# cgranerob/Land-Surface-Temperature-Super-Resolution-with-a-Scale-Invariance-Free-Neural-Approach

Measured on AMD Instinct MI355X. Metric: LST+NDVI 256x256 patches/sec (train fwd+bwd), whole job, higher is better.
Workload: dtype f32; 1 GPU; ModelB SIF-NN-SR2 (gradFTM loss) batch 64/GPU, synthetic 256x256, 1x MI355X, fwd+loss+bwd+Adam; batch_per_gpu=64, patch=256x256 (LST 64x64 + NDVI 256x256), parallelism=dp1, loss=sr2

## Files before the change

land-surface-temperature-super-resolution-with-a-scale-invariance-free-neural-approach_amd/csrc/edge_conv.h:

```cpp
#pragma once
#include "common.h"

int conv_in_fwd_blocks(int B, int H, int W);
int launch_conv_in_fwd(const float* x, const float* w, float* y, float* partials, int B, int H, int W, hipStream_t s,
                       int* nf_image = nullptr);
int launch_conv_in_wgrad(const float* x, const float* dy, float* partials, int nblk, float* dw, int B, int H, int W, hipStream_t s);
int launch_conv_out_fwd(const float* y, const float* scale, const float* shift, const float* w, const float* bias,
                        float* out, int B, int H, int W, hipStream_t s,
                        const int* nf = nullptr);
int launch_conv_out_dgrad(const float* dsr, const float* w, float* g, int B, int H, int W, hipStream_t s);
int launch_conv_out_wgrad(const float* y, const float* scale, const float* shift, const float* dsr, float* partials,
                          int nblk, float* dw, float* db, int B, int H, int W, hipStream_t s);
int launch_conv_in_wgrad_fused(const float* x, const float* g, const float* y, const float* scale, const float* shift,
                               const double* coef, float* partials, int nblk, float* dw, int B, int H, int W, hipStream_t s);
size_t conv_in_gram_scratch_floats();
int launch_conv_in_gram(const float* x, float* scratch, int B, int H, int W, hipStream_t s);
const double* conv_in_gram_result(const float* scratch);
int launch_conv_in_dz_wgrad(const float* x, const float* dz, float* partials, int nblk, int B, int H, int W, hipStream_t s);
int launch_conv_in_dw_combine(const float* partials, int nblk, const double* gram, const float* w, const double* coef, float* dw,
                              hipStream_t s);
int launch_tail_bwd_reduce(const float* y, const float* scale, const float* shift, const float* mean, const float* invstd,
                           const float* dsr, const float* w, float* wpart, float* bnpart, int nblk, int B, int H, int W,
                           hipStream_t s, int* nf = nullptr);
int launch_tail_bwd_apply(const float* y, const float* scale, const float* shift, const double* coef, const float* dsr,
                          const float* w, float* dy, int B, int H, int W, hipStream_t s);
int launch_sum_partials(const float* partials, int nblk, int n, float* out, hipStream_t s);

int launch_bn_finalize(const float* partials, int nblk, int C, double count, const float* gamma, const float* beta,
                       float* run_mean, float* run_var, float momentum, float eps, float* mean, float* invstd,
                       float* scale, float* shift, hipStream_t s,
                       int* nf = nullptr);
int launch_bn_eval_coeffs(const float* params, const float* running, float eps, float* scale, float* shift, hipStream_t s,
                          int* nf = nullptr, const int* nf_pack = nullptr);
int launch_bn_bwd_reduce(const float* g, const float* y, const float* scale, const float* shift, const float* mean,
                         const float* invstd, int C, size_t npix, float* partials, int nblk, hipStream_t s,
                         const float* gp = nullptr, int H = 0, int W = 0, float* g_out = nullptr);
int launch_bn_bwd_finalize(const float* partials, int nblk, int C, double count, const float* scale, const float* mean,
                           const float* invstd, float* dgamma, float* dbeta, double* coef, hipStream_t s,
                           const float* shift = nullptr, const float* beta = nullptr, float* coef_f = nullptr,
                           const float* xs_partials = nullptr, int xs_n = 0, float* xs_out = nullptr,
                           int frozen = 0,
                           const int* nf = nullptr);
int launch_bn_bwd_finalize2(const float* pa, int na, const float* pb, int nb, int C, double count, const float* scale,
                            const float* mean, const float* invstd, float* dgamma, float* dbeta, double* coef, hipStream_t s,
                            const float* shift = nullptr, const float* beta = nullptr, float* coef_f = nullptr, int frozen = 0,
                            const int* nf = nullptr);
int launch_bn_bwd_apply(const float* g, const float* y, const float* scale, const float* shift, const double* coef,
                        int C, size_t npix, float* dy, hipStream_t s, const float* gp = nullptr, int H = 0, int W = 0);
int launch_nbt_increment(long long* nbt, int n, hipStream_t s);

int launch_bn_frozen_stats(const float* running, float eps, float* mean, float* invstd, hipStream_t s);
int launch_conv_in_dgrad(const float* g, const float* y, const float* scale, const float* shift, const double* coef, const float* w,
                         float* dx, int B, int H, int W, hipStream_t s);

int launch_bnrelu_pool2(const float* y, const float* scale, const float* shift, float* out, int B, int H, int W, int C, hipStream_t s);
int launch_bnrelu_add(const float* p, const float* y, const float* scale, const float* shift, float* out, int C, size_t npix, hipStream_t s);
int launch_bnrelu_up2x(const float* y, const float* scale, const float* shift, float* out, int B, int Hin, int Win, int C, hipStream_t s);
int launch_pool2_bwd(const float* gp, float* g, int B, int H, int W, int C, int accumulate, hipStream_t s);
int launch_up2x_bwd(const float* gu, float* g, int B, int Hin, int Win, int C, hipStream_t s, const float* bn_y = nullptr,
                    const float* bn_scale = nullptr, const float* bn_shift = nullptr, float* bn_partials = nullptr);
int up2x_bwd_stat_rows(int B, int Hin, int Win, int C);

int launch_adam_flat(float* p, const float* g, float* m, float* v, int n, float lr, float beta1, float beta2, float eps,
                     float weight_decay, int step, float grad_scale, hipStream_t s);

int launch_adam_flat_dev(float* p, const float* g, float* m, float* v, int n, float lr, float beta1, float beta2, float eps,
                         float weight_decay, long long* step_dev, float* coef2, float grad_scale, hipStream_t s);

int launch_tiles_prepare(const float* lst, const float* ndvi, float* x, int T, int tiles_x, int win, long long lst_step_y,
                         long long lst_step_x, int lst_row, long long ndvi_step_y, long long ndvi_step_x, int ndvi_row,
                         float mean_lst, float std_lst, float mean_ndvi, float std_ndvi, int clip_ndvi, hipStream_t s);
int launch_tiles_paste(const float* sr, float* out, int T, int tiles_x, int hr, long long out_row, float mean, float std,
                       hipStream_t s);
int launch_l4pool4(const float* x, float* out, int B, int H, int W, hipStream_t s);
size_t psnr_ssim_scratch_bytes(int B, int H, int W);
int launch_psnr_ssim(const float* pred, const float* targ, int B, int H, int W, void* scratch, float* out2, hipStream_t s);
size_t psnr_ssim_masked_scratch_bytes(int B, int H, int W);
int launch_psnr_ssim_masked(const float* pred, const float* targ, const unsigned char* valid, int scale, int B, int H, int W,
                            void* scratch, float* out2, int* counts2, hipStream_t s);

size_t eval_metrics_scratch_bytes(int B, int H, int W);
int launch_eval_metrics(const float* a, const float* b, int B, int H, int W, const float* taps9, float data_range,
                        void* scratch, double* out8, hipStream_t s);
int launch_gradient_strata(const float* a, int B, int H, int W, const float* taps9, float* g, float* q2, int* counts3,
                           hipStream_t s);
size_t eval_metrics_masked_scratch_bytes(int B, int H, int W);
int launch_eval_metrics_masked(const float* a, const float* b, const unsigned char* mask, int B, int H, int W,
                               const float* taps9, float data_range, void* scratch, double* out8, int* counts5, hipStream_t s);

size_t fourier_scratch_bytes(int B, int H, int W);
int launch_fft2_attenuation(const float* img, int B, int H, int W, void* scratch, float* mag, float* spectrum, hipStream_t s);
```

land-surface-temperature-super-resolution-with-a-scale-invariance-free-neural-approach_amd/csrc/edge_conv.hip:

```cpp
#include "edge_conv.h"

namespace {

template <bool HS>
__global__ __launch_bounds__(256) void conv_in_fwd_kernel(const float* __restrict__ x, const float* __restrict__ w,
                                                          float* __restrict__ y, float* __restrict__ partials,
                                                          int B, int H, int W, int* __restrict__ nf_image) {
  __shared__ float tile[2][2 * 324];
  __shared__ float red[4][16][2];
  const int tid = threadIdx.x, lane = tid & 63, wave = tid >> 6;
  const int i = lane & 15, kq = lane >> 4;
  const int tiles_x = (W + 15) / 16, tiles_y = (H + 15) / 16, ntiles = B * tiles_x * tiles_y;
  auto stage = [&](int t, float* dst) {
    const int tx = t % tiles_x, ty = (t / tiles_x) % tiles_y, b = t / (tiles_x * tiles_y);
    const int x0 = tx * 16, y0 = ty * 16;
    for (int e = tid; e < 2 * 324; e += 256) {
      const int c = e / 324, p = e - c * 324;
      const int py = p / 18, px = p - py * 18;
      const int gy = clampi(y0 - 1 + py, 0, H - 1), gx = clampi(x0 - 1 + px, 0, W - 1);
      dst[e] = x[((size_t)(b * 2 + c) * H + gy) * W + gx];
    }
  };
  if ((int)blockIdx.x < ntiles) stage(blockIdx.x, tile[0]);
  float wa[5];
  int off[5];
#pragma unroll
  for (int j = 0; j < 5; ++j) {
    const int kk = 4 * j + kq;
    wa[j] = kk < 18 ? w[i * 18 + kk] : 0.f;
    const int c = kk >= 9 ? 1 : 0, t = kk < 18 ? kk - 9 * c : 0;
    off[j] = (kk < 18 ? c * 324 : 0) + (t / 3) * 18 + t % 3 + i;
  }
  float s1[4] = {0.f, 0.f, 0.f, 0.f}, s2[4] = {0.f, 0.f, 0.f, 0.f};
  int buf = 0;
  for (int t = blockIdx.x; t < ntiles; t += gridDim.x, buf ^= 1) {
    __syncthreads();
    if (t + (int)gridDim.x < ntiles) stage(t + gridDim.x, tile[buf ^ 1]);
    const int tx = t % tiles_x, ty = (t / tiles_x) % tiles_y, b = t / (tiles_x * tiles_y);
    const int x0 = tx * 16, y0 = ty * 16;
    const float* T = tile[buf];
    bool bad = false;
#pragma unroll
    for (int r = 0; r < 4; ++r) {
      const int row = 4 * wave + r;
      f32x4 acc = (f32x4){0.f, 0.f, 0.f, 0.f};
#pragma unroll
      for (int j = 0; j < 5; ++j) acc = __builtin_amdgcn_mfma_f32_16x16x4f32(wa[j], T[off[j] + row * 18], acc, 0, 0, 0);
      if (y0 + row < H && x0 + i < W) {
        const float4 o = as_stored4<HS>(make_float4(acc[0], acc[1], acc[2], acc[3]));
        stA4<HS>(y, ((size_t)(b * H + y0 + row) * W + x0 + i) * 16 + 4 * kq, o);
        const float ov[4] = {o.x, o.y, o.z, o.w};
#pragma unroll
        for (int q = 0; q < 4; ++q) { s1[q] += ov[q]; s2[q] = fmaf(ov[q], ov[q], s2[q]); bad = bad || nonfinite(ov[q]); }
      }
    }
    if (nf_image != nullptr && bad) nf_image[b] = 1;
  }
  if (partials != nullptr) {
#pragma unroll
    for (int q = 0; q < 4; ++q) {
#pragma unroll
      for (int m = 1; m < 16; m <<= 1) { s1[q] += __shfl_xor(s1[q], m); s2[q] += __shfl_xor(s2[q], m); }
      if (i == 0) { red[wave][4 * kq + q][0] = s1[q]; red[wave][4 * kq + q][1] = s2[q]; }
    }
    __syncthreads();
    if (tid < 32) {
      const int co = tid >> 1, j = tid & 1;
      const float s = red[0][co][j] + red[1][co][j] + red[2][co][j] + red[3][co][j];
      partials[((size_t)blockIdx.x * 16 + co) * 2 + j] = s;
    }
  }
}

template <bool FUSED, bool HS>
__global__ __launch_bounds__(256) void conv_in_wgrad_kernel(const float* __restrict__ x, const float* __restrict__ dy,
                                                            const float* __restrict__ yraw,
                                                            const float* __restrict__ scale,
                                                            const float* __restrict__ shift,
                                                            const double* __restrict__ coef,
                                                            float* __restrict__ partials, int B, int H, int W) {
  SIFSR_CHAIN_PRIO();
  __shared__ float tile[2 * 324 + 8];
  __shared__ float dyt[256 * 16];
  __shared__ float red[4][2][256];
  const int tid = threadIdx.x, lane = tid & 63, wave = tid >> 6;
  const int tiles_x = (W + 15) / 16, tiles_y = (H + 15) / 16, ntiles = B * tiles_x * tiles_y;
  const int i16 = lane & 15, k = lane >> 4;
  int offn[2];
#pragma unroll
  for (int nt = 0; nt < 2; ++nt) {
    const int n = nt * 16 + i16;
    offn[nt] = n < 18 ? (n / 9) * 324 + ((n % 9) / 3) * 18 + (n % 9) % 3 : 0;
  }
  f32x4 acc[2] = {(f32x4){0.f, 0.f, 0.f, 0.f}, (f32x4){0.f, 0.f, 0.f, 0.f}};
  float4 sc4, sh4;
  double sd[4], k1[4], k0[4];
  if (FUSED) {
    const int q4 = tid & 3;
    sc4 = ld4(scale + 4 * q4); sh4 = ld4(shift + 4 * q4);
#pragma unroll
    for (int j = 0; j < 4; ++j) { sd[j] = coef[4 * q4 + j]; k1[j] = coef[16 + 4 * q4 + j]; k0[j] = coef[32 + 4 * q4 + j]; }
  }
  for (int tl = blockIdx.x; tl < ntiles; tl += gridDim.x) {
    const int tx = tl % tiles_x, ty = (tl / tiles_x) % tiles_y, b = tl / (tiles_x * tiles_y);
    const int x0 = tx * 16, y0 = ty * 16;
    __syncthreads();
    for (int e = tid; e < 2 * 324; e += 256) {
      const int c = e / 324, p = e - c * 324;
      const int py = p / 18, px = p - py * 18;
      const int gy = clampi(y0 - 1 + py, 0, H - 1), gx = clampi(x0 - 1 + px, 0, W - 1);
      tile[e] = x[((size_t)(b * 2 + c) * H + gy) * W + gx];
    }
    for (int e = tid; e < 256 * 4; e += 256) {
      const int p = e >> 2, c4 = e & 3;
      if (y0 + (p >> 4) >= H || x0 + (p & 15) >= W) {
        *reinterpret_cast<float4*>(&dyt[p * 16 + 4 * c4]) = make_float4(0.f, 0.f, 0.f, 0.f);
        continue;
      }
      const size_t off = ((size_t)(b * H + y0 + (p >> 4)) * W + x0 + (p & 15)) * 16 + 4 * c4;
      float4 v = ldA4<HS>(dy, off);
      if (FUSED) {
        const float4 yv = ldA4<HS>(yraw, off);
        v.x = (float)fma(sd[0], (double)(fmaf(yv.x, sc4.x, sh4.x) > 0.f ? v.x : 0.f), fma(k1[0], (double)yv.x, k0[0]));
        v.y = (float)fma(sd[1], (double)(fmaf(yv.y, sc4.y, sh4.y) > 0.f ? v.y : 0.f), fma(k1[1], (double)yv.y, k0[1]));
        v.z = (float)fma(sd[2], (double)(fmaf(yv.z, sc4.z, sh4.z) > 0.f ? v.z : 0.f), fma(k1[2], (double)yv.z, k0[2]));
        v.w = (float)fma(sd[3], (double)(fmaf(yv.w, sc4.w, sh4.w) > 0.f ? v.w : 0.f), fma(k1[3], (double)yv.w, k0[3]));
      }
      *reinterpret_cast<float4*>(&dyt[p * 16 + 4 * c4]) = v;
    }
    __syncthreads();
#pragma unroll 4
    for (int ks = wave; ks < 64; ks += 4) {
      const int r = ks >> 2, qd = ks & 3;
      const float av = dyt[(r * 16 + 4 * qd + k) * 16 + i16];
      const int base = r * 18 + 4 * qd + k;
      acc[0] = __builtin_amdgcn_mfma_f32_16x16x4f32(av, tile[offn[0] + base], acc[0], 0, 0, 0);
      acc[1] = __builtin_amdgcn_mfma_f32_16x16x4f32(av, tile[offn[1] + base], acc[1], 0, 0, 0);
    }
  }
#pragma unroll
  for (int nt = 0; nt < 2; ++nt)
#pragma unroll
    for (int r = 0; r < 4; ++r) red[wave][nt][(4 * k + r) * 16 + i16] = acc[nt][r];
  __syncthreads();
  for (int e = tid; e < 288; e += 256) {
    const int co = e / 18, n = e % 18;
    const int nt = n >> 4, col = n & 15;
    partials[(size_t)blockIdx.x * 288 + e] =
        red[0][nt][co * 16 + col] + red[1][nt][co * 16 + col] + red[2][nt][co * 16 + col] + red[3][nt][co * 16 + col];
  }
}

constexpr int OCS = 20;

template <bool HS>
__global__ __launch_bounds__(256) void conv_out_fwd_kernel(const float* __restrict__ y, const float* scale,
                                                           const float* shift, const float* __restrict__ w,
                                                           const float* __restrict__ bias, float* __restrict__ out,
                                                           int H, int W, const int* __restrict__ nf) {
  constexpr int NGRP = 21;
  __shared__ float P[NGRP * 16 * 9];
  const int tid = threadIdx.x, lane = tid & 63, wave = tid >> 6;
  const int i = lane & 15, kq = lane >> 4;
  const int x0 = blockIdx.x * 16, y0 = blockIdx.y * 16, b = blockIdx.z;
  const int poisoned = nf != nullptr ? (nf[NF_BATCH] | nf[NF_IMAGE + b]) : 0;
  float wb[4];
#pragma unroll
  for (int j = 0; j < 4; ++j) wb[j] = i < 9 ? w[(4 * kq + j) * 9 + i] : 0.f;
  float4 sc = make_float4(1.f, 1.f, 1.f, 1.f), sh = make_float4(0.f, 0.f, 0.f, 0.f);
  if (scale != nullptr) { sc = ld4(scale + 4 * kq); sh = ld4(shift + 4 * kq); }
  constexpr int NPW = (NGRP + 3) / 4;
  float4 v[NPW];
#pragma unroll
  for (int n = 0; n < NPW; ++n) {
    const int g = wave + 4 * n;
    int p = g * 16 + i;
    if (p > 323) p = 323;
    const int r = p / 18, c = p - r * 18;
    const int gy = clampi(y0 - 1 + r, 0, H - 1), gx = clampi(x0 - 1 + c, 0, W - 1);
    v[n] = ldA4<HS>(y, ((size_t)(b * H + gy) * W + gx) * 16 + 4 * kq);
  }
#pragma unroll
  for (int n = 0; n < NPW; ++n) {
    const int g = wave + 4 * n;
    if (g >= NGRP) break;
    float4 a = v[n];
    if (scale != nullptr) a = bn_relu4(a, sc, sh);
    f32x4 acc = (f32x4){0.f, 0.f, 0.f, 0.f};
    acc = __builtin_amdgcn_mfma_f32_16x16x4f32(a.x, wb[0], acc, 0, 0, 0);
    acc = __builtin_amdgcn_mfma_f32_16x16x4f32(a.y, wb[1], acc, 0, 0, 0);
    acc = __builtin_amdgcn_mfma_f32_16x16x4f32(a.z, wb[2], acc, 0, 0, 0);
    acc = __builtin_amdgcn_mfma_f32_16x16x4f32(a.w, wb[3], acc, 0, 0, 0);
    if (i < 9) {
#pragma unroll
      for (int r = 0; r < 4; ++r) P[(g * 16 + 4 * kq + r) * 9 + i] = acc[r];
    }
  }
  __syncthreads();
  const int ty = tid >> 4, tx = tid & 15;
  float s = bias[0];
#pragma unroll
  for (int t = 0; t < 9; ++t) s += P[((ty + t / 3) * 18 + tx + t % 3) * 9 + t];
  if (poisoned != 0) s = __uint_as_float(0x7fc00000u);
  if (y0 + ty < H && x0 + tx < W) out[(size_t)(b * H + y0 + ty) * W + x0 + tx] = s;
}

template <bool HS>
__global__ __launch_bounds__(256) void conv_out_dgrad_kernel(const float* __restrict__ dsr, const float* __restrict__ w,
                                                             float* __restrict__ g, int B, int H, int W) {
  const size_t n = (size_t)B * H * W;
  for (size_t q = (size_t)blockIdx.x * blockDim.x + threadIdx.x; q < n; q += (size_t)gridDim.x * blockDim.x) {
    const int qx = q % W, qy = (q / W) % H;
    const size_t img = q - (size_t)qy * W - qx;
    float S[9];
#pragma unroll
    for (int t = 0; t < 9; ++t) {
      const int ty = t / 3 - 1, tx = t % 3 - 1;
      int ys[2], ny = 0, xs[2], nx = 0;
      if (qy - ty >= 0 && qy - ty < H) ys[ny++] = qy - ty;
      if ((qy == 0 && ty == -1) || (qy == H - 1 && ty == 1)) ys[ny++] = qy;
      if (qx - tx >= 0 && qx - tx < W) xs[nx++] = qx - tx;
      if ((qx == 0 && tx == -1) || (qx == W - 1 && tx == 1)) xs[nx++] = qx;
      float s = 0.f;
      for (int iy = 0; iy < ny; ++iy)
        for (int ix = 0; ix < nx; ++ix) s += dsr[img + (size_t)ys[iy] * W + xs[ix]];
      S[t] = s;
    }
#pragma unroll
    for (int c4 = 0; c4 < 4; ++c4) {
      float o[4];
#pragma unroll
      for (int j = 0; j < 4; ++j) {
        float s = 0.f;
#pragma unroll
        for (int t = 0; t < 9; ++t) s = fmaf(w[(4 * c4 + j) * 9 + t], S[t], s);
        o[j] = s;
      }
      stA4<HS>(g, q * 16 + 4 * c4, make_float4(o[0], o[1], o[2], o[3]));
    }
  }
}

template <bool HS>
__global__ __launch_bounds__(256) void conv_out_wgrad_kernel(const float* __restrict__ y, const float* scale,
                                                             const float* shift, const float* __restrict__ dsr,
                                                             float* __restrict__ partials, int B, int H, int W) {
  __shared__ float tile[18 * 20 * OCS];
  __shared__ float dt[256];
  __shared__ float red[4][256];
  __shared__ float bsum[4];
  const int tid = threadIdx.x, lane = tid & 63, wave = tid >> 6;
  const int tiles_x = (W + 15) / 16, tiles_y = (H + 15) / 16, ntiles = B * tiles_x * tiles_y;
  const int i16 = lane & 15, k = lane >> 4;
  const int tty = i16 < 9 ? i16 / 3 : 100, ttx = i16 < 9 ? i16 % 3 : 100;
  f32x4 acc = (f32x4){0.f, 0.f, 0.f, 0.f};
  float bacc = 0.f;
  for (int e = tid; e < 18 * 20 * OCS; e += 256) tile[e] = 0.f;
  for (int tl = blockIdx.x; tl < ntiles; tl += gridDim.x) {
    const int tx = tl % tiles_x, ty = (tl / tiles_x) % tiles_y, b = tl / (tiles_x * tiles_y);
    const int x0 = tx * 16, y0 = ty * 16;
    __syncthreads();
    for (int e = tid; e < 324 * 4; e += 256) {
      const int p = e >> 2, c4 = e & 3;
      const int py = p / 18, px = p - py * 18;
      const int gy = clampi(y0 - 1 + py, 0, H - 1), gx = clampi(x0 - 1 + px, 0, W - 1);
      float4 v = ldA4<HS>(y, ((size_t)(b * H + gy) * W + gx) * 16 + 4 * c4);
      if (scale != nullptr) v = bn_relu4(v, ld4(scale + 4 * c4), ld4(shift + 4 * c4));
      *reinterpret_cast<float4*>(&tile[(py * 20 + px) * OCS + 4 * c4]) = v;
    }
    const float dv = (y0 + (tid >> 4) < H && x0 + (tid & 15) < W) ? dsr[(size_t)(b * H + y0 + (tid >> 4)) * W + x0 + (tid & 15)] : 0.f;
    dt[tid] = dv;
    bacc += dv;
    __syncthreads();
    for (int ks = wave; ks < 90; ks += 4) {
      const int row = ks / 5, col = (ks - row * 5) * 4 + k;
      const float av = tile[(row * 20 + col) * OCS + i16];
      const int oy = row - tty, ox = col - ttx;
      const float bv = (oy >= 0 && oy < 16 && ox >= 0 && ox < 16) ? dt[oy * 16 + ox] : 0.f;
      acc = __builtin_amdgcn_mfma_f32_16x16x4f32(av, bv, acc, 0, 0, 0);
    }
  }
#pragma unroll
  for (int r = 0; r < 4; ++r) red[wave][(4 * k + r) * 16 + i16] = acc[r];
#pragma unroll
  for (int m = 1; m < 64; m <<= 1) bacc += __shfl_xor(bacc, m);
  if (lane == 0) bsum[wave] = bacc;
  __syncthreads();
  if (tid < 144) {
    const int ci = tid / 9, t = tid % 9;
    partials[(size_t)blockIdx.x * 145 + tid] = red[0][ci * 16 + t] + red[1][ci * 16 + t] + red[2][ci * 16 + t] + red[3][ci * 16 + t];
  } else if (tid == 144) {
    partials[(size_t)blockIdx.x * 145 + 144] = bsum[0] + bsum[1] + bsum[2] + bsum[3];
  }
}

constexpr int GRAM_N = 189, GRAM_PITCH = 192;
__host__ __device__ constexpr int gram_idx(int kr, int k) { return kr * 18 - kr * (kr - 1) / 2 + (k - kr); }

template <int WV> static __device__ __forceinline__ void gram_rows(const float (&pv)[20], f32x2 (&acc)[26]) {
  int n = 0;
#pragma unroll
  for (int kr = WV; kr < 18; kr += 4)
#pragma unroll
    for (int k = kr; k < 18; k += 2) { acc[n] = __builtin_elementwise_fma((f32x2){pv[kr], pv[kr]}, (f32x2){pv[k], pv[k + 1]}, acc[n]); ++n; }
}
template <int WV> static __device__ __forceinline__ void gram_store(const f32x2 (&acc)[26], float* __restrict__ row, int lane) {
  int n = 0;
#pragma unroll
  for (int kr = WV; kr < 18; kr += 4)
#pragma unroll
    for (int k = kr; k < 18; k += 2) {
#pragma unroll
      for (int h = 0; h < 2; ++h) {
        float v = acc[n][h];
#pragma unroll
        for (int m = 1; m < 64; m <<= 1) v += __shfl_xor(v, m);
        if (lane == 0 && k + h < 18) row[gram_idx(kr, k + h)] = v;
      }
      ++n;
    }
}

template <bool FULL>
__global__ __launch_bounds__(256, 2) void conv_in_gram_kernel(const float* __restrict__ x, float* __restrict__ partials, int B, int H, int W) {
  __shared__ float tile[2][2 * 324 + 8];
  const int tid = threadIdx.x, lane = tid & 63;
  const int wave = __builtin_amdgcn_readfirstlane(tid >> 6);
  const int tiles_x = (W + 15) / 16, tiles_y = (H + 15) / 16, ntiles = B * tiles_x * tiles_y;
  float px_[3];
  auto fetch = [&](int t) __attribute__((always_inline)) {
    const int tx = t % tiles_x, ty = (t / tiles_x) % tiles_y, b = t / (tiles_x * tiles_y);
    const int x0 = tx * 16, y0 = ty * 16;
#pragma unroll
    for (int i = 0; i < 3; ++i) {
      const int e = min(tid + 256 * i, 2 * 324 - 1);
      const int c = e / 324, p = e - c * 324;
      const int py = p / 18, pxx = p - py * 18;
      px_[i] = x[((size_t)(b * 2 + c) * H + clampi(y0 - 1 + py, 0, H - 1)) * W + clampi(x0 - 1 + pxx, 0, W - 1)];
    }
  };
  f32x2 acc[26], xs[9];
#pragma unroll
  for (int i = 0; i < 26; ++i) acc[i] = (f32x2){0.f, 0.f};
#pragma unroll
  for (int i = 0; i < 9; ++i) xs[i] = (f32x2){0.f, 0.f};
  if ((int)blockIdx.x < ntiles) fetch(blockIdx.x);
  int buf = 0;
  for (int t = blockIdx.x; t < ntiles; t += gridDim.x, buf ^= 1) {
    tile[buf][tid] = px_[0];
    tile[buf][tid + 256] = px_[1];
    if (tid + 512 < 2 * 324) tile[buf][tid + 512] = px_[2];
    __syncthreads();
    fetch(t + (int)gridDim.x < ntiles ? t + (int)gridDim.x : t);
    const int tx = t % tiles_x, ty = (t / tiles_x) % tiles_y;
    const int x0 = tx * 16, y0 = ty * 16;
    const float* T = tile[buf];
#pragma unroll 1
    for (int i = 0; i < 4; ++i) {
      const int r = (lane >> 4) + 4 * i, col = lane & 15;
      const bool inside = FULL || (y0 + r < H && x0 + col < W);
      float pv[20];
#pragma unroll
      for (int k = 0; k < 18; ++k) {
        const float v = T[(k / 9) * 324 + (r + (k % 9) / 3) * 18 + col + (k % 9) % 3];
        pv[k] = inside ? v : 0.f;
      }
      pv[18] = pv[19] = 0.f;
      switch (wave) {
        case 0: gram_rows<0>(pv, acc); break;
        case 1: gram_rows<1>(pv, acc); break;
        case 2: gram_rows<2>(pv, acc); break;
        default:
          gram_rows<3>(pv, acc);
#pragma unroll
          for (int k = 0; k < 9; ++k) xs[k] += (f32x2){pv[2 * k], pv[2 * k + 1]};
      }
    }
  }
  float* row = partials + (size_t)blockIdx.x * GRAM_PITCH;
  switch (wave) {
    case 0: gram_store<0>(acc, row, lane); break;
    case 1: gram_store<1>(acc, row, lane); break;
    case 2: gram_store<2>(acc, row, lane); break;
    default:
      gram_store<3>(acc, row, lane);
#pragma unroll
      for (int k = 0; k < 18; ++k) {
        float v = xs[k >> 1][k & 1];
#pragma unroll
        for (int m = 1; m < 64; m <<= 1) v += __shfl_xor(v, m);
        if (lane == 0) row[171 + k] = v;
      }
  }
}

__global__ __launch_bounds__(64) void conv_in_gram_reduce_kernel(const float* __restrict__ partials, int nblk, double* __restrict__ gram) {
  const int e = blockIdx.x, lane = threadIdx.x;
  double s = 0.0;
  for (int k = lane; k < nblk; k += 64) s += (double)partials[(size_t)k * GRAM_PITCH + e];
#pragma unroll
  for (int m = 32; m > 0; m >>= 1) s += __shfl_xor(s, m);
  if (lane == 0) gram[e] = s;
}

template <bool HS>
__global__ __launch_bounds__(256, 3) void conv_in_dz_wgrad_kernel(const float* __restrict__ x, const float* __restrict__ dz,
                                                                  float* __restrict__ partials, int B, int H, int W) {
  SIFSR_CHAIN_PRIO();
  __shared__ float tile[2][2 * 324 + 8];
  __shared__ float red[4][4][72];
  const int tid = threadIdx.x, lane = tid & 63, wave = tid >> 6;
  const int tiles_x = (W + 15) / 16, tiles_y = (H + 15) / 16, ntiles = B * tiles_x * tiles_y;
  const int c4 = tid & 3, pl = tid >> 2;
  const int lx = pl & 15, ly0 = pl >> 4;
  f32x2 acc[4][9];
#pragma unroll
  for (int j = 0; j < 4; ++j)
#pragma unroll
    for (int u = 0; u < 9; ++u) acc[j][u] = (f32x2){0.f, 0.f};
  float4 pz[4];
  float px_[3];
  size_t nbase = 0;
  int nrow[4] = {0, 0, 0, 0};
  bool nin[4] = {false, false, false, false};
  auto fetch_z = [&](int k) __attribute__((always_inline)) { pz[k] = ldA4<HS>(dz, nbase + (size_t)nrow[k]); };
  auto fetch = [&](int tl) __attribute__((always_inline)) {
    const int tx = tl % tiles_x, r = tl / tiles_x, ty = r % tiles_y, b = r / tiles_y;
    const int x0 = tx * 16, y0 = ty * 16;
    const int gx = min(x0 + lx, W - 1);
    nbase = ((size_t)(b * H) * W + gx) * 16 + 4 * c4;
#pragma unroll
    for (int k = 0; k < 4; ++k) {
      nrow[k] = min(y0 + ly0 + 4 * k, H - 1) * W * 16;
      nin[k] = y0 + ly0 + 4 * k < H && x0 + lx < W;
    }
#pragma unroll
    for (int i = 0; i < 3; ++i) {
      const int e = min(tid + 256 * i, 2 * 324 - 1);
      const int c = e / 324, p = e - c * 324;
      const int py = p / 18, pxx = p - py * 18;
      px_[i] = x[((size_t)(b * 2 + c) * H + clampi(y0 - 1 + py, 0, H - 1)) * W + clampi(x0 - 1 + pxx, 0, W - 1)];
    }
  };
  int buf = 0;
  bool cin_[4] = {false, false, false, false};
  if ((int)blockIdx.x < ntiles) {
    fetch(blockIdx.x);
#pragma unroll
    for (int k = 0; k < 4; ++k) fetch_z(k);
  }
  for (int tl = blockIdx.x; tl < ntiles; tl += gridDim.x, buf ^= 1) {
    tile[buf][tid] = px_[0];
    tile[buf][tid + 256] = px_[1];
    if (tid + 512 < 2 * 324) tile[buf][tid + 512] = px_[2];
#pragma unroll
    for (int k = 0; k < 4; ++k) cin_[k] = nin[k];
    __syncthreads();
    fetch(tl + (int)gridDim.x < ntiles ? tl + (int)gridDim.x : tl);
    const float* T = tile[buf];
#pragma unroll
    for (int k = 0; k < 4; ++k) {
      float4 zv = pz[k];
      fetch_z(k);
      __builtin_amdgcn_sched_barrier(0);
      if (!cin_[k]) zv = make_float4(0.f, 0.f, 0.f, 0.f);
      const int ly = ly0 + 4 * k;
      f32x2 pp[9];
#pragma unroll
      for (int u = 0; u < 9; ++u) {
        const int n0 = 2 * u, n1 = 2 * u + 1;
        pp[u] = (f32x2){T[(n0 / 9) * 324 + (ly + (n0 % 9) / 3) * 18 + lx + (n0 % 9) % 3],
                        T[(n1 / 9) * 324 + (ly + (n1 % 9) / 3) * 18 + lx + (n1 % 9) % 3]};
      }
      const float zz[4] = {zv.x, zv.y, zv.z, zv.w};
#pragma unroll
      for (int j = 0; j < 4; ++j)
#pragma unroll
        for (int u = 0; u < 9; ++u) acc[j][u] = __builtin_elementwise_fma((f32x2){zz[j], zz[j]}, pp[u], acc[j][u]);
    }
  }
#pragma unroll
  for (int j = 0; j < 4; ++j)
#pragma unroll
    for (int u = 0; u < 9; ++u)
#pragma unroll
      for (int h = 0; h < 2; ++h) {
        float v = acc[j][u][h];
#pragma unroll
        for (int m = 4; m < 64; m <<= 1) v += __shfl_xor(v, m);
        if (lane < 4) red[wave][c4][j * 18 + 2 * u + h] = v;
      }
  __syncthreads();
  for (int e = tid; e < 288; e += 256) {
    const int co = e / 18, n = e - co * 18;
    const int q = co >> 2, i = (co & 3) * 18 + n;
    partials[(size_t)blockIdx.x * 288 + e] = red[0][q][i] + red[1][q][i] + red[2][q][i] + red[3][q][i];
  }
}

__global__ __launch_bounds__(64) void conv_in_dw_combine_kernel(const float* __restrict__ partials, int nblk,
                                                                const double* __restrict__ gram, const float* __restrict__ w,
                                                                const double* __restrict__ coef, float* __restrict__ dw) {
  const int e = blockIdx.x, lane = threadIdx.x;
  const int c = e / 18, k = e - c * 18;
  double s = 0.0;
  for (int r = lane; r < nblk; r += 64) s += (double)partials[(size_t)r * 288 + e];
#pragma unroll
  for (int m = 32; m > 0; m >>= 1) s += __shfl_xor(s, m);
  if (lane == 0) {
    double a = 0.0;
    for (int kr = 0; kr < 18; ++kr) a += (double)w[c * 18 + kr] * gram[kr <= k ? gram_idx(kr, k) : gram_idx(k, kr)];
    dw[e] = (float)(coef[c] * s + coef[16 + c] * a + coef[32 + c] * gram[171 + k]);
  }
}

__global__ __launch_bounds__(256) void sum_partials_kernel(const float* __restrict__ partials, int nblk, int n,
                                                           float* __restrict__ out) {
  __shared__ double part[64][4];
  const int el = threadIdx.x & 3, grp = threadIdx.x >> 2;
  const int e = blockIdx.x * 4 + el;
  double s = 0.0;
  if (e < n)
    for (int k = grp; k < nblk; k += 64) s += (double)partials[(size_t)k * n + e];
  part[grp][el] = s;
  __syncthreads();
  for (int st = 32; st > 0; st >>= 1) {
    if (grp < st) part[grp][el] += part[grp + st][el];
    __syncthreads();
  }
  if (grp == 0 && e < n) out[e] = (float)part[0][el];
}

}

int conv_in_fwd_blocks(int B, int H, int W) {
  const int ntiles = B * ((H + 15) / 16) * ((W + 15) / 16);
  return ntiles < 2048 ? ntiles : 2048;
}

int launch_conv_in_fwd(const float* x, const float* w, float* y, float* partials, int B, int H, int W, hipStream_t s, int* nf_image) {
  if (H < 1 || W < 1 || B < 1) return SIFSR_ERR_SHAPE;
  if (sifsr_half_storage()) hipLaunchKernelGGL(conv_in_fwd_kernel<true>, dim3(conv_in_fwd_blocks(B, H, W)), dim3(256), 0, s, x, w, y, partials, B, H, W, nf_image);
  else hipLaunchKernelGGL(conv_in_fwd_kernel<false>, dim3(conv_in_fwd_blocks(B, H, W)), dim3(256), 0, s, x, w, y, partials, B, H, W, nf_image);
  SIFSR_LAUNCH_CHECK();
  return SIFSR_OK;
}

int launch_conv_in_wgrad(const float* x, const float* dy, float* partials, int nblk, float* dw, int B, int H, int W,
                         hipStream_t s) {
  if (H < 1 || W < 1) return SIFSR_ERR_SHAPE;
  if (sifsr_half_storage()) hipLaunchKernelGGL((conv_in_wgrad_kernel<false, true>), dim3(nblk), dim3(256), 0, s, x, dy, nullptr, nullptr, nullptr, nullptr, partials, B, H, W);
  else hipLaunchKernelGGL((conv_in_wgrad_kernel<false, false>), dim3(nblk), dim3(256), 0, s, x, dy, nullptr, nullptr, nullptr, nullptr, partials, B, H, W);
  hipLaunchKernelGGL(sum_partials_kernel, dim3(72), dim3(256), 0, s, partials, nblk, 288, dw);
  SIFSR_LAUNCH_CHECK();
  return SIFSR_OK;
}

int launch_conv_in_wgrad_fused(const float* x, const float* g, const float* y, const float* scale, const float* shift,
                               const double* coef, float* partials, int nblk, float* dw, int B, int H, int W,
                               hipStream_t s) {
  if (H < 1 || W < 1) return SIFSR_ERR_SHAPE;
  if (sifsr_half_storage()) hipLaunchKernelGGL((conv_in_wgrad_kernel<true, true>), dim3(nblk), dim3(256), 0, s, x, g, y, scale, shift, coef, partials, B, H, W);
  else hipLaunchKernelGGL((conv_in_wgrad_kernel<true, false>), dim3(nblk), dim3(256), 0, s, x, g, y, scale, shift, coef, partials, B, H, W);
  hipLaunchKernelGGL(sum_partials_kernel, dim3(72), dim3(256), 0, s, partials, nblk, 288, dw);
  SIFSR_LAUNCH_CHECK();
  return SIFSR_OK;
}

size_t conv_in_gram_scratch_floats() { return (size_t)1024 * GRAM_PITCH + 2 * GRAM_PITCH; }
int launch_conv_in_gram(const float* x, float* scratch, int B, int H, int W, hipStream_t s) {
  if (H < 1 || W < 1 || B < 1) return SIFSR_ERR_SHAPE;
  const int ntiles = B * ((H + 15) / 16) * ((W + 15) / 16);
  const int nblk = ntiles < 512 ? ntiles : 512;
  if (H % 16 == 0 && W % 16 == 0) hipLaunchKernelGGL(conv_in_gram_kernel<true>, dim3(nblk), dim3(256), 0, s, x, scratch, B, H, W);
  else hipLaunchKernelGGL(conv_in_gram_kernel<false>, dim3(nblk), dim3(256), 0, s, x, scratch, B, H, W);
  hipLaunchKernelGGL(conv_in_gram_reduce_kernel, dim3(GRAM_N), dim3(64), 0, s, scratch, nblk, reinterpret_cast<double*>(scratch + (size_t)1024 * GRAM_PITCH));
  SIFSR_LAUNCH_CHECK();
  return SIFSR_OK;
}
const double* conv_in_gram_result(const float* scratch) { return reinterpret_cast<const double*>(scratch + (size_t)1024 * GRAM_PITCH); }

int launch_conv_in_dz_wgrad(const float* x, const float* dz, float* partials, int nblk, int B, int H, int W, hipStream_t s) {
  if (H < 1 || W < 1 || nblk < 1) return SIFSR_ERR_SHAPE;
  if (sifsr_half_storage()) hipLaunchKernelGGL(conv_in_dz_wgrad_kernel<true>, dim3(nblk), dim3(256), 0, s, x, dz, partials, B, H, W);
  else hipLaunchKernelGGL(conv_in_dz_wgrad_kernel<false>, dim3(nblk), dim3(256), 0, s, x, dz, partials, B, H, W);
  SIFSR_LAUNCH_CHECK();
  return SIFSR_OK;
}
int launch_conv_in_dw_combine(const float* partials, int nblk, const double* gram, const float* w, const double* coef, float* dw,
                              hipStream_t s) {
  hipLaunchKernelGGL(conv_in_dw_combine_kernel, dim3(288), dim3(64), 0, s, partials, nblk, gram, w, coef, dw);
  SIFSR_LAUNCH_CHECK();
  return SIFSR_OK;
}

int launch_conv_out_fwd(const float* y, const float* scale, const float* shift, const float* w, const float* bias,
                        float* out, int B, int H, int W, hipStream_t s, const int* nf) {
  if (H < 1 || W < 1) return SIFSR_ERR_SHAPE;
  if (sifsr_half_storage()) hipLaunchKernelGGL(conv_out_fwd_kernel<true>, dim3((W + 15) / 16, (H + 15) / 16, B), dim3(256), 0, s, y, scale, shift, w, bias, out, H, W, nf);
  else hipLaunchKernelGGL(conv_out_fwd_kernel<false>, dim3((W + 15) / 16, (H + 15) / 16, B), dim3(256), 0, s, y, scale, shift, w, bias, out, H, W, nf);
  SIFSR_LAUNCH_CHECK();
  return SIFSR_OK;
}

int launch_conv_out_dgrad(const float* dsr, const float* w, float* g, int B, int H, int W, hipStream_t s) {
  const size_t n = (size_t)B * H * W;
  int blocks = (int)((n + 255) / 256);
  if (blocks > 8192) blocks = 8192;
  if (sifsr_half_storage()) hipLaunchKernelGGL(conv_out_dgrad_kernel<true>, dim3(blocks), dim3(256), 0, s, dsr, w, g, B, H, W);
  else hipLaunchKernelGGL(conv_out_dgrad_kernel<false>, dim3(blocks), dim3(256), 0, s, dsr, w, g, B, H, W);
  SIFSR_LAUNCH_CHECK();
  return SIFSR_OK;
}

int launch_conv_out_wgrad(const float* y, const float* scale, const float* shift, const float* dsr, float* partials,
                          int nblk, float* dw, float* db, int B, int H, int W, hipStream_t s) {
  if (H < 1 || W < 1) return SIFSR_ERR_SHAPE;
  if (sifsr_half_storage()) hipLaunchKernelGGL(conv_out_wgrad_kernel<true>, dim3(nblk), dim3(256), 0, s, y, scale, shift, dsr, partials, B, H, W);
  else hipLaunchKernelGGL(conv_out_wgrad_kernel<false>, dim3(nblk), dim3(256), 0, s, y, scale, shift, dsr, partials, B, H, W);
  if (db != dw + 144) return SIFSR_ERR_ARG;
  hipLaunchKernelGGL(sum_partials_kernel, dim3(37), dim3(256), 0, s, partials, nblk, 145, dw);
  SIFSR_LAUNCH_CHECK();
  return SIFSR_OK;
}

int launch_sum_partials(const float* partials, int nblk, int n, float* out, hipStream_t s) {
  hipLaunchKernelGGL(sum_partials_kernel, dim3((n + 3) / 4), dim3(256), 0, s, partials, nblk, n, out);
  SIFSR_LAUNCH_CHECK();
  return SIFSR_OK;
}
```

land-surface-temperature-super-resolution-with-a-scale-invariance-free-neural-approach_amd/csrc/engine.hip:

```cpp
#include "engine.h"
#include "switches.h"

#include <stdio.h>
#include <stdlib.h>

#include <mutex>
#include <vector>

static thread_local bool t_half_storage = false;
bool sifsr_half_storage() { return t_half_storage; }
HalfStorageScope::HalfStorageScope(bool on) : prev(t_half_storage) { t_half_storage = on; }
HalfStorageScope::~HalfStorageScope() { t_half_storage = prev; }

static int env_int(const char* name, int dflt) { const char* v = getenv(name); return v ? atoi(v) : dflt; }
const Switches& sifsr_switches() {
  static const Switches sw = {
      env_int("SIFSR_WGRAD_STREAM", 1), env_int("SIFSR_WGRAD_WINO", 2),  env_int("SIFSR_NO_WINO", 0),
      env_int("SIFSR_NO_WINO8", 0),     env_int("SIFSR_NO_BWD16", 0),    env_int("SIFSR_TAIL_APPLY", 0),
      env_int("SIFSR_HEAD_LINEAR", 0),  env_int("SIFSR_BF16_BWD16", 0),  env_int("SIFSR_DBG_EARLY_REDUCE", 3),
      env_int("SIFSR_DBG_POOL_ON_LOAD", 1)};
  return sw;
}

static constexpr int enc_prev[3] = {L_IN3, L_D1C, L_D2C};
static constexpr int enc_a[3] = {L_D1A, L_D2A, L_D3A}, enc_b[3] = {L_D1B, L_D2B, L_D3B}, enc_c[3] = {L_D1C, L_D2C, L_D3C};
static constexpr int pc[3] = {16, 32, 64};
static constexpr int dec_low[3] = {L_D3C, L_U1B, L_U2B}, dec_skip[3] = {L_D2C, L_D1C, L_IN3};
static constexpr int dec_a[3] = {L_U1A, L_U2A, L_U3A}, dec_b[3] = {L_U1B, L_U2B, L_U3B};
static constexpr int uc[3] = {64, 32, 16};

static NetTable build_net() {
  static const int cin[SIFSR_NUM_BN_LAYERS] = {2, 16, 16, 16, 16, 32, 32, 32, 64, 64, 64, 128, 64, 64, 32, 32, 16};
  static const int cout[SIFSR_NUM_BN_LAYERS] = {16, 16, 16, 16, 32, 32, 32, 64, 64, 64, 64, 64, 32, 32, 16, 16, 16};
  static const int level[SIFSR_NUM_BN_LAYERS] = {0, 0, 1, 1, 1, 2, 2, 2, 3, 3, 3, 2, 2, 1, 1, 0, 0};
  NetTable t;
  int p = 0, r = 0, c = 0, wp = 0;
  for (int l = 0; l < SIFSR_NUM_BN_LAYERS; ++l) {
    LayerInfo& L = t.L[l];
    L.cin = cin[l]; L.cout = cout[l]; L.level = level[l];
    L.w_off = p; p += cout[l] * cin[l] * 9;
    L.gamma_off = p; p += cout[l];
    L.beta_off = p; p += cout[l];
    L.run_off = r; r += 2 * cout[l];
    L.ch_off = c; c += cout[l];
    L.wpack_off = wp;
    if (l > 0) wp += 9 * cin[l] * cout[l];
  }
  t.out_w_off = p; p += 144;
  t.out_b_off = p; p += 1;
  t.total_params = p; t.total_running = r; t.total_channels = c; t.total_wpack = wp;
  return t;
}
const NetTable& sifsr_net() {
  static const NetTable t = build_net();
  return t;
}

static size_t align64(size_t n) { return (n + 63) & ~(size_t)63; }

static int wgrad_blocks(int cin, int cout, int chunks, int ntiles, bool wino) {
  const int total = wino ? (cout == 64 ? 256 : 512) : (cin == 16 && cout == 16 ? 1536 : 768);
  int n = total / chunks;
  if (n < 64) n = 64;
  const int cap = ntiles / 4 > 0 ? ntiles / 4 : 1;
  if (n > cap) n = cap;
  return n;
}

int sifsr_layout(int B, int H, int W, int training, WsLayout* o) {
  if (B < 1 || H < 24 || W < 24 || H % 8 || W % 8) return SIFSR_ERR_SHAPE;
  const NetTable& nt = sifsr_net();
  WsLayout& w = *o;
  size_t off = 0;
  auto take = [&](size_t n) { const size_t r = off; off += align64(n); return r; };
  size_t N[4];
  N[0] = (size_t)B * H * W; N[1] = N[0] / 4; N[2] = N[0] / 16; N[3] = N[0] / 64;
  for (int i = 0; i < 4; ++i) w.npix[i] = N[i];

  w.mean = take(nt.total_channels); w.invstd = take(nt.total_channels);
  w.scale = take(nt.total_channels); w.shift = take(nt.total_channels);
  w.nf = take(NF_IMAGE + (size_t)B + NF_PACK_WORDS);
  w.wfwd = take(nt.total_wpack); w.wdg = take(4 * (size_t)nt.total_wpack);
  w.wwf = take((size_t)nt.total_wpack / 9 * 16); w.wwd = take((size_t)nt.total_wpack / 9 * 16);
  for (int l = 0; l < SIFSR_NUM_BN_LAYERS; ++l) w.y[l] = take(nt.L[l].cout * N[nt.L[l].level]);
  for (int k = 0; k < 3; ++k) {
    w.P[k] = take(pc[k] * N[k + 1]);
    w.R[k] = take(pc[k] * N[k + 1]);
  }
  for (int k = 0; k < 3; ++k) w.U[k] = take(uc[k] * N[2 - k]);

  size_t maxpart = 0;
  for (int l = 0; l < SIFSR_NUM_BN_LAYERS; ++l) {
    const int lh = H >> nt.L[l].level, lw = W >> nt.L[l].level;
    const size_t nblk = (size_t)B * ((lh + 15) / 16) * ((lw + 15) / 16);
    const size_t n = (nblk > 1024 ? nblk : 1024) * nt.L[l].cout * 2;
    maxpart = n > maxpart ? n : maxpart;
  }
  for (int k = 0; k < 3; ++k) {
    const int lh = H >> (3 - k), lw = W >> (3 - k);
    const size_t n = (size_t)up2x_bwd_stat_rows(B, lh, lw, uc[k]) * uc[k] * 2;
    maxpart = n > maxpart ? n : maxpart;
  }
  w.partials = take(maxpart);
  w.partials_cap = maxpart;
  w.fwd_end = off;
  if (training) {
    w.coef = take(6 * 64);
    w.coef_f = take(4 * (size_t)nt.total_channels);
    w.bpart = take((size_t)dgrad_border_waves(B, H, W, 16) * 32);
    for (int l = 0; l < SIFSR_NUM_BN_LAYERS; ++l) w.g[l] = take(nt.L[l].cout * N[nt.L[l].level]);
    w.dy_border = take(16 * N[0]);
    w.dyB[0] = w.dyB[1] = w.dyB[2] = w.dy_border;
    for (int k = 0; k < 3; ++k) w.gP[k] = take(pc[k] * N[k + 1]);
    for (int k = 0; k < 3; ++k) w.gU[k] = take(uc[k] * N[2 - k]);
    w.slabs = take(1024 * 288);
    w.gram = take(conv_in_gram_scratch_floats());
    w.slab_l[0] = 0; w.slab_cap[0] = 0;
    for (int l = 1; l < SIFSR_NUM_BN_LAYERS; ++l) {
      const int lvh = H >> nt.L[l].level, lvw = W >> nt.L[l].level;
      const int ntiles = B * ((lvh + 7) / 8) * ((lvw + 15) / 16);
      const int nb_tap = wgrad_blocks(nt.L[l].cin, nt.L[l].cout, 1, ntiles, false), nb_wino = wgrad_blocks(nt.L[l].cin, nt.L[l].cout, 1, ntiles, true);
      w.slab_cap[l] = (size_t)(nb_tap > nb_wino ? nb_tap : nb_wino) * 9 * nt.L[l].cin * nt.L[l].cout;
      if (nt.L[l].cin == 16 && nt.L[l].cout == 16 && conv3x3_bwd16_applies(B, lvh, lvw)) {
        const size_t need = (size_t)conv3x3_bwd16_grid(B, lvh, lvw) * 9 * 256;
        if (need > w.slab_cap[l]) w.slab_cap[l] = need;
      }
      w.slab_l[l] = take(w.slab_cap[l]);
    }
  }
  w.total = off;
  return SIFSR_OK;
}

namespace {

struct Ctx {
  const NetTable& nt;
  WsLayout lay;
  float* ws;
  const float* params;
  int B, H, W;
  hipStream_t s;
  int bf16 = 0;
  int frozen = 0;
  float* grads = nullptr;
  struct BwdState* bwd = nullptr;
  struct SideLane* side = nullptr;
  bool* forked = nullptr;
  int lvH(int lv) const { return H >> lv; }
  int lvW(int lv) const { return W >> lv; }
  float* f(size_t off) const { return ws + off; }
  float* y(int l) const { return ws + lay.y[l]; }
  float* g(int l) const { return ws + lay.g[l]; }
  float* mean(int l) const { return ws + lay.mean + nt.L[l].ch_off; }
  float* invstd(int l) const { return ws + lay.invstd + nt.L[l].ch_off; }
  float* scale(int l) const { return ws + lay.scale + nt.L[l].ch_off; }
  float* shift(int l) const { return ws + lay.shift + nt.L[l].ch_off; }
  float* coef_f(int l) const { return ws + lay.coef_f + 4 * (size_t)nt.L[l].ch_off; }
  double* coef() const { return reinterpret_cast<double*>(ws + lay.coef); }
  float* slab(int l) const { return ws + lay.slab_l[l]; }
  int* nf() const { return reinterpret_cast<int*>(ws + lay.nf); }
  size_t wn(int l) const { return (size_t)9 * nt.L[l].cin * nt.L[l].cout; }
  const float* w_dgrad_f32(int l) const { return ws + lay.wdg + 4 * (size_t)nt.L[l].wpack_off; }
  const float* w_fwd(int l) const { return bf16 ? w_dgrad_f32(l) + wn(l) : ws + lay.wfwd + nt.L[l].wpack_off; }
  const float* w_dgrad(int l) const { return bf16 ? w_dgrad_f32(l) + wn(l) + wn(l) / 2 : w_dgrad_f32(l); }
  const float* w_fwd_wino(int l) const { return ws + lay.wwf + (size_t)nt.L[l].wpack_off / 9 * 16; }
  const float* w_dgrad_wino(int l) const { return ws + lay.wwd + (size_t)nt.L[l].wpack_off / 9 * 16; }
};

struct BwdState {
  WgradReduceJob jobs[16];
  int njobs = 0;
  int last_fused = -1;
};

ConvSrc src_raw(const float* p, int C) { ConvSrc s; s.ptr = p; s.scale = nullptr; s.shift = nullptr; s.C = C; s.coff = 0; s.nq = C / 16; return s; }
ConvSrc src_act(const Ctx& c, int l) {
  ConvSrc s; s.ptr = c.y(l); s.scale = c.scale(l); s.shift = c.shift(l); s.C = c.nt.L[l].cout; s.coff = 0; s.nq = s.C / 16; return s;
}
ConvSrc src_none() { ConvSrc s; s.ptr = nullptr; s.scale = nullptr; s.shift = nullptr; s.C = 0; s.coff = 0; s.nq = 0; return s; }

#define SIFSR_TRY(expr) do { int rc__ = (expr); if (rc__ != SIFSR_OK) return rc__; } while (0)

struct SideLane {
  hipStream_t s = nullptr;
  hipEvent_t ev[SIFSR_NUM_BN_LAYERS] = {};
  hipEvent_t join = nullptr;
  hipEvent_t aux = nullptr;
  bool ok = false;
  std::mutex in_use;
};

int g_side_override = -1;

SideLane* side_lane(hipStream_t main_stream) {
  if (!(g_side_override >= 0 ? g_side_override : sifsr_switches().wgrad_stream)) return nullptr;
  static std::mutex mu;
  static SideLane lanes[16];
  static bool tried[16] = {};
  int dev = 0;
  if (hipGetDevice(&dev) != hipSuccess || dev < 0 || dev >= 16) return nullptr;
  hipStreamCaptureStatus cap = hipStreamCaptureStatusNone;
  if (hipStreamIsCapturing(main_stream, &cap) != hipSuccess) { (void)hipGetLastError(); return nullptr; }
  if (cap != hipStreamCaptureStatusNone) return nullptr;
  if (main_stream != nullptr) {
    hipDevice_t sdev = -1;
    if (hipStreamGetDevice(main_stream, &sdev) != hipSuccess || (int)sdev != dev) { (void)hipGetLastError(); return nullptr; }
  }
  std::lock_guard<std::mutex> lk(mu);
  SideLane& L = lanes[dev];
  if (!tried[dev]) {
    tried[dev] = true;
    int lo = 0, hi = 0;
    (void)hipDeviceGetStreamPriorityRange(&lo, &hi);
    bool ok = hipStreamCreateWithPriority(&L.s, hipStreamNonBlocking, lo) == hipSuccess;
    for (int i = 0; ok && i < SIFSR_NUM_BN_LAYERS; ++i) ok = hipEventCreateWithFlags(&L.ev[i], hipEventDisableTiming) == hipSuccess;
    ok = ok && hipEventCreateWithFlags(&L.join, hipEventDisableTiming) == hipSuccess;
    ok = ok && hipEventCreateWithFlags(&L.aux, hipEventDisableTiming) == hipSuccess;
    L.ok = ok;
    (void)hipGetLastError();
  }
  return L.ok ? &L : nullptr;
}

struct SideLaneGuard {
  SideLane* lane; hipStream_t main; bool forked = false, joined = false;
  SideLaneGuard(SideLane* l, hipStream_t m) : lane(l), main(m) { if (lane) lane->in_use.lock(); }
  int join() {
    if (!lane || joined) return SIFSR_OK;
    joined = true;
    if (!forked) return SIFSR_OK;
    if (hipEventRecord(lane->join, lane->s) != hipSuccess || hipStreamWaitEvent(main, lane->join, 0) != hipSuccess) return SIFSR_ERR_ARG;
    return SIFSR_OK;
  }
  ~SideLaneGuard() { if (lane) { (void)join(); lane->in_use.unlock(); } }
};

constexpr int PROF_SLOTS = 24;
constexpr size_t PROF_POOL = 1024;
struct ProfSlot {
  int layer = -1, phase = 0;
  std::vector<hipEvent_t> start, stop;
  size_t used = 0;
};
struct ProfState {
  ProfSlot slot[PROF_SLOTS];
  int active = 0;
  std::mutex mu;
};
ProfState g_prof;

struct ProfScope {
  hipStream_t s; int sl = -1; long idx = -1;
  ProfScope(int layer, int phase, hipStream_t st) : s(st) {
    if (g_prof.active == 0) return;
    std::lock_guard<std::mutex> lk(g_prof.mu);
    for (int k = 0; k < g_prof.active; ++k) {
      ProfSlot& p = g_prof.slot[k];
      if (p.layer == layer && p.phase == phase && p.used < p.start.size()) {
        sl = k; idx = (long)p.used++;
        (void)hipEventRecord(p.start[idx], s);
        return;
      }
    }
  }
  ~ProfScope() {
    if (idx < 0) return;
    std::lock_guard<std::mutex> lk(g_prof.mu);
    ProfSlot& p = g_prof.slot[sl];
    if ((size_t)idx < p.stop.size()) (void)hipEventRecord(p.stop[idx], s);
  }
};

int bn_unit_finalize(const Ctx& c, int l, int nblk, float* running, float momentum, float eps) {
  const LayerInfo& L = c.nt.L[l];
  return launch_bn_finalize(c.f(c.lay.partials), nblk, L.cout, (double)c.lay.npix[L.level], c.params + L.gamma_off,
                            c.params + L.beta_off, running + L.run_off, running + L.run_off + L.cout, momentum, eps,
                            c.mean(l), c.invstd(l), c.scale(l), c.shift(l), c.s, c.nf());
}

int conv_unit_fwd(const Ctx& c, int l, ConvSrc s0, ConvSrc s1, int training, float* running, float momentum, float eps) {
  const LayerInfo& L = c.nt.L[l];
  ConvArgs a;
  a.src[0] = s0; a.src[1] = s1;
  a.dst[0].ptr = c.y(l); a.dst[0].C = L.cout; a.dst[0].coff = 0;
  a.dst[1] = a.dst[0];
  a.bf16 = c.bf16;
  a.wpack = c.w_fwd(l);
  a.wpack_wino = c.w_fwd_wino(l);
  a.addend = nullptr; a.addC = 0;
  a.stat_partials = training ? c.f(c.lay.partials) : nullptr;
  a.dst_split = L.cout / 16;
  a.B = c.B; a.H = c.lvH(L.level); a.W = c.lvW(L.level);
  a.NQ = L.cin / 16;
  {
    ProfScope ps(l, 1, c.s);
    SIFSR_TRY(launch_conv3x3_mfma(a, L.cout, 0, c.s));
  }
  if (training)
    SIFSR_TRY(bn_unit_finalize(c, l, conv3x3_grid_blocks(c.B, a.H, a.W, L.cout, conv3x3_wino_kind(a, L.cout, 0)), running, momentum, eps));
  return SIFSR_OK;
}

int bn_bwd_reduce_blocks(size_t npix) {
  const size_t nb = npix / 256;
  return (int)(nb > 1024 ? 1024 : (nb < 1 ? 1 : nb));
}
int bn_unit_bwd(const Ctx& c, int l, const float* gp = nullptr, int fused_stats = 0, int border_rows = -1,
                bool writeback = true) {
  const LayerInfo& L = c.nt.L[l];
  const int lh = c.lvH(L.level), lw = c.lvW(L.level);
  const size_t npix = c.lay.npix[L.level];
  float* dgamma = c.grads + L.gamma_off, *dbeta = c.grads + L.beta_off;
  if (fused_stats > 0) {
    if (gp != nullptr) return SIFSR_ERR_ARG;
    return launch_bn_bwd_finalize2(c.f(c.lay.partials), fused_stats, c.f(c.lay.bpart), border_rows >= 0 ? border_rows : dgrad_border_waves(c.B, lh, lw, 16),
                                   L.cout, (double)npix, c.scale(l), c.mean(l), c.invstd(l), dgamma, dbeta, c.coef(), c.s, c.shift(l),
                                   c.params + L.beta_off, c.coef_f(l), c.frozen, c.nf());
  }
  const int nblk = bn_bwd_reduce_blocks(npix);
  SIFSR_TRY(launch_bn_bwd_reduce(c.g(l), c.y(l), c.scale(l), c.shift(l), c.mean(l), c.invstd(l), L.cout, npix, c.f(c.lay.partials), nblk,
                                 c.s, gp, lh, lw, (gp && writeback) ? c.g(l) : nullptr));
  return launch_bn_bwd_finalize(c.f(c.lay.partials), nblk, L.cout, (double)npix, c.scale(l), c.mean(l), c.invstd(l), dgamma, dbeta,
                                c.coef(), c.s, c.shift(l), c.params + L.beta_off, c.coef_f(l), nullptr, 0, nullptr, c.frozen, c.nf());
}

static bool wgrad_wino_policy(int cout) {
  const int mode = sifsr_switches().wgrad_wino;
  return mode == 2 || (mode == 1 && cout <= 32);
}

int conv_unit_wgrad(const Ctx& c, int l, ConvSrc s0, ConvSrc s1, const float* dy, bool dy_stored = false) {
  const LayerInfo& L = c.nt.L[l];
  WgradArgs a;
  a.src[0] = s0; a.src[1] = s1;
  a.dy = dy; a.slabs = c.slab(l);
  if (!dy_stored) { a.dy_y = c.y(l); a.dy_coef = c.coef_f(l); }
  a.B = c.B; a.H = c.lvH(L.level); a.W = c.lvW(L.level);
  a.NQ = L.cin / 16;
  a.ntiles = c.B * ((a.H + 7) / 8) * ((a.W + 15) / 16);
  a.bf16 = c.bf16;
  const bool wino = wgrad_wino_policy(L.cout) && conv3x3_wgrad_use_wino(a, L.cin, L.cout);
  const int nbi = wino ? wgrad_wino_nbi_chunk(L.cin) : wgrad_nbi_chunk(a, L.cin);
  const int nblk = wgrad_blocks(L.cin, L.cout, L.cin / (16 * nbi), a.ntiles, wino);
  if ((size_t)nblk * (L.cin / (16 * nbi)) * 9 * (16 * nbi) * L.cout > c.lay.slab_cap[l]) return SIFSR_ERR_WORKSPACE;
  hipStream_t ws = c.s;
  if (c.side != nullptr) {
    if (hipEventRecord(c.side->ev[l], c.s) != hipSuccess || hipStreamWaitEvent(c.side->s, c.side->ev[l], 0) != hipSuccess)
      return SIFSR_ERR_ARG;
    ws = c.side->s;
    *c.forked = true;
  }
  {
    ProfScope ps(l, 3, ws);
    if (wino) SIFSR_TRY(launch_conv3x3_wgrad_wino(a, L.cin, L.cout, nblk, ws));
    else SIFSR_TRY(launch_conv3x3_wgrad(a, L.cin, L.cout, nblk, ws));
  }
  WgradReduceJob& j = c.bwd->jobs[c.bwd->njobs++];
  j.slab_off = c.lay.slab_l[l]; j.nblk = nblk; j.cin = L.cin; j.cout = L.cout; j.nbi_chunk = nbi; j.w_off = L.w_off;
  return SIFSR_OK;
}

int conv_unit_dgrad(const Ctx& c, int l, const float* dy, float* g0, int C0, int split_ch, float* g1, int C1,
                    const float* addend, int bn_layer = -1, int* stat_rows = nullptr, bool dy_stored = false) {
  const LayerInfo& L = c.nt.L[l];
  const bool fuse = bn_layer >= 0 && L.cin == 16 && C0 == 16 && split_ch == 16 && g1 == nullptr && addend == nullptr &&
                    c.nt.L[bn_layer].cout == 16 && c.nt.L[bn_layer].level == L.level;
  if (stat_rows) *stat_rows = 0;
  ConvArgs a;
  a.src[0] = src_raw(dy, L.cout); a.src[1] = src_none();
  const float* dy_edge = dy;
  if (!dy_stored) {
    a.bw_y = c.y(l); a.bw_coef = c.coef_f(l); a.bw_border = c.f(c.lay.dy_border);
    dy_edge = a.bw_border;
  }
  a.dst[0].ptr = g0; a.dst[0].C = C0; a.dst[0].coff = 0;
  a.dst[1].ptr = g1 ? g1 : g0; a.dst[1].C = g1 ? C1 : C0; a.dst[1].coff = 0;
  a.bf16 = c.bf16;
  a.wpack = c.w_dgrad(l);
  a.wpack_wino = c.w_dgrad_wino(l);
  a.addend = addend; a.addC = L.cin;
  a.stat_partials = nullptr;
  a.dst_split = split_ch / 16;
  a.B = c.B; a.H = c.lvH(L.level); a.W = c.lvW(L.level);
  a.NQ = L.cout / 16;
  if (fuse) {
    a.stat_partials = c.f(c.lay.partials);
    a.bn_y = c.y(bn_layer); a.bn_scale = c.scale(bn_layer); a.bn_shift = c.shift(bn_layer);
    if (stat_rows) *stat_rows = conv3x3_grid_blocks(c.B, a.H, a.W, L.cin, conv3x3_wino_kind(a, L.cin, 1));
  }
  {
    ProfScope ps(l, 2, c.s);
    SIFSR_TRY(launch_conv3x3_mfma(a, L.cin, 1, c.s));
  }
  SIFSR_TRY(launch_dgrad_border_fix(dy_edge, L.cout, c.w_dgrad_f32(l), L.cin, g0, C0, split_ch, g1 ? g1 : g0, g1 ? C1 : C0, c.B, a.H,
                                    a.W, c.s, c.bf16, fuse ? a.bn_y : nullptr, fuse ? a.bn_scale : nullptr,
                                    fuse ? a.bn_shift : nullptr, fuse ? c.f(c.lay.bpart) : nullptr));
  return SIFSR_OK;
}

bool bwd16_usable(const Ctx& c, int l, ConvSrc s0) {
  const LayerInfo& L = c.nt.L[l];
  return L.cin == 16 && L.cout == 16 && (c.bf16 == 0 || sifsr_switches().bf16_bwd16) && wgrad_wino_policy(16) && s0.C == 16 &&
         s0.coff == 0 && conv3x3_bwd16_applies(c.B, c.lvH(L.level), c.lvW(L.level));
}
int conv_unit_bwd16(const Ctx& c, int l, ConvSrc s0, const float* dy, float* gin, const float* addend, int bn_layer, int* stat_rows,
                    int dy_mode, bool* applied, bool store_dz = false, const float* pool_gp = nullptr) {
  const LayerInfo& L = c.nt.L[l];
  *applied = false;
  if (stat_rows) *stat_rows = 0;
  const int lh = c.lvH(L.level), lw = c.lvW(L.level);
  if (!bwd16_usable(c, l, s0)) return dy_mode == 2 ? SIFSR_ERR_ARG : SIFSR_OK;
  const bool dy_stored = dy_mode == 0;
  const bool fuse = bn_layer >= 0 && addend == nullptr && c.nt.L[bn_layer].cout == 16 && c.nt.L[bn_layer].level == L.level;
  const int grid = conv3x3_bwd16_grid(c.B, lh, lw);
  if ((size_t)grid * 9 * 256 > c.lay.slab_cap[l] || (fuse && (size_t)grid * 32 > c.lay.partials_cap)) return SIFSR_ERR_WORKSPACE;
  Bwd16Args a;
  a.x = s0.ptr; a.x_scale = s0.scale; a.x_shift = s0.shift;
  if (dy_mode == 2) { a.tail_dsr = dy; a.tail_w = c.params + c.nt.out_w_off; }
  else a.g = dy;
  if (!dy_stored) { a.y = c.y(l); a.coef = c.coef_f(l); a.dy_border = c.f(c.lay.dy_border); }
  a.wpack_wino = c.w_dgrad_wino(l);
  a.gin = gin; a.addend = addend;
  if (fuse) {
    a.bn_y = c.y(bn_layer); a.bn_scale = c.scale(bn_layer); a.bn_shift = c.shift(bn_layer); a.stat_partials = c.f(c.lay.partials);
    if (stat_rows) *stat_rows = grid;
  }
  a.slabs = c.slab(l);
  a.B = c.B; a.H = lh; a.W = lw;
  a.half = c.bf16;
  if (store_dz && !fuse) return SIFSR_ERR_ARG;
  a.store_dz = store_dz ? 1 : 0;
  a.pool_gp = pool_gp;
  {
    ProfScope ps(l, 2, c.s);
    SIFSR_TRY(launch_conv3x3_bwd16(a, c.s));
  }
  SIFSR_TRY(launch_dgrad_border_fix(dy_stored ? dy : a.dy_border, 16, c.w_dgrad_f32(l), 16, gin, 16, 16, gin, 16, c.B, lh, lw, c.s, c.bf16,
                                    fuse ? a.bn_y : nullptr, fuse ? a.bn_scale : nullptr, fuse ? a.bn_shift : nullptr,
                                    fuse ? c.f(c.lay.bpart) : nullptr, a.store_dz));
  WgradReduceJob& j = c.bwd->jobs[c.bwd->njobs++];
  j.slab_off = c.lay.slab_l[l]; j.nblk = grid; j.cin = 16; j.cout = 16; j.nbi_chunk = 1; j.w_off = L.w_off;
  if (c.side != nullptr && hipEventRecord(c.side->ev[l], c.s) != hipSuccess) return SIFSR_ERR_ARG;
  c.bwd->last_fused = l;
  *applied = true;
  return SIFSR_OK;
}

int conv_unit_bwd(const Ctx& c, int l, ConvSrc s0, const float* dy, float* gin, const float* addend, int bn_layer, int* stat_rows,
                  int dy_mode = 1) {
  bool fused = false;
  SIFSR_TRY(conv_unit_bwd16(c, l, s0, dy, gin, addend, bn_layer, stat_rows, dy_mode, &fused));
  if (fused) return SIFSR_OK;
  const int cin = c.nt.L[l].cin;
  SIFSR_TRY(conv_unit_wgrad(c, l, s0, src_none(), dy, dy_mode == 0));
  return conv_unit_dgrad(c, l, dy, gin, cin, cin, nullptr, 0, addend, bn_layer, stat_rows, dy_mode == 0);
}

int finish_wgrads(const Ctx& c, hipStream_t st) {
  BwdState& b = *c.bwd;
  if (b.njobs > 0) SIFSR_TRY(launch_wgrad_reduce_batched(c.ws, b.jobs, b.njobs, c.grads, st));
  b.njobs = 0;
  return SIFSR_OK;
}
int finish_wgrads_side(const Ctx& c) {
  if (c.bwd->last_fused >= 0) {
    if (hipStreamWaitEvent(c.side->s, c.side->ev[c.bwd->last_fused], 0) != hipSuccess) return SIFSR_ERR_ARG;
    *c.forked = true;
  }
  return finish_wgrads(c, c.side->s);
}

}

int sifsr_engine_forward(const float* x, float* sr, const float* params, float* running, long long* nbt, float* ws,
                         size_t ws_floats, int B, int H, int W, int training, float momentum, float eps,
                         hipStream_t s, int bf16) {
  if (!x || !sr || !params || !running || !ws) return SIFSR_ERR_ARG;
  Ctx c{sifsr_net(), WsLayout(), ws, params, B, H, W, s};
  if (bf16 < 0 || bf16 > 1) return SIFSR_ERR_ARG;
  c.bf16 = bf16;
  const HalfStorageScope storage(bf16 == 1);
  SIFSR_TRY(sifsr_layout(B, H, W, training, &c.lay));
  if (ws_floats < c.lay.fwd_end) return SIFSR_ERR_WORKSPACE;
  const NetTable& nt = c.nt;
  const WsLayout& w = c.lay;

  SIFSR_TRY(launch_pack_weights(params, c.f(w.wfwd), c.f(w.wdg), s, c.f(w.wwf), c.f(w.wwd), training ? nbt : nullptr, SIFSR_NUM_BN_LAYERS,
                                c.nf(), NF_IMAGE + B));
  if (!training) {
    SIFSR_TRY(launch_bn_eval_coeffs(params, running, eps, c.f(w.scale), c.f(w.shift), s, c.nf(), c.nf() + NF_IMAGE + B));
  }

  SIFSR_TRY(launch_conv_in_fwd(x, params + nt.L[L_IN0].w_off, c.y(L_IN0), training ? c.f(w.partials) : nullptr, B, H, W, s,
                               c.nf() + NF_IMAGE));
  if (training) SIFSR_TRY(bn_unit_finalize(c, L_IN0, conv_in_fwd_blocks(B, H, W), running, momentum, eps));
  SIFSR_TRY(conv_unit_fwd(c, L_IN3, src_act(c, L_IN0), src_none(), training, running, momentum, eps));

  for (int k = 0; k < 3; ++k) {
    const int lp = enc_prev[k];
    SIFSR_TRY(launch_bnrelu_pool2(c.y(lp), c.scale(lp), c.shift(lp), c.f(w.P[k]), B, c.lvH(k), c.lvW(k), pc[k], s));
    SIFSR_TRY(conv_unit_fwd(c, enc_a[k], src_raw(c.f(w.P[k]), pc[k]), src_none(), training, running, momentum, eps));
    SIFSR_TRY(conv_unit_fwd(c, enc_b[k], src_act(c, enc_a[k]), src_none(), training, running, momentum, eps));
    SIFSR_TRY(launch_bnrelu_add(c.f(w.P[k]), c.y(enc_b[k]), c.scale(enc_b[k]), c.shift(enc_b[k]), c.f(w.R[k]), pc[k],
                                w.npix[k + 1], s));
    SIFSR_TRY(conv_unit_fwd(c, enc_c[k], src_raw(c.f(w.R[k]), pc[k]), src_none(), training, running, momentum, eps));
  }

  for (int k = 0; k < 3; ++k) {
    const int lv = 2 - k;
    const int ll = dec_low[k];
    SIFSR_TRY(launch_bnrelu_up2x(c.y(ll), c.scale(ll), c.shift(ll), c.f(w.U[k]), B, c.lvH(lv + 1), c.lvW(lv + 1), uc[k], s));
    SIFSR_TRY(conv_unit_fwd(c, dec_a[k], src_raw(c.f(w.U[k]), uc[k]), src_act(c, dec_skip[k]), training, running, momentum, eps));
    SIFSR_TRY(conv_unit_fwd(c, dec_b[k], src_act(c, dec_a[k]), src_none(), training, running, momentum, eps));
  }

  SIFSR_TRY(launch_conv_out_fwd(c.y(L_U3B), c.scale(L_U3B), c.shift(L_U3B), params + nt.out_w_off,
                                params + nt.out_b_off, sr, B, H, W, s, c.nf()));
  return SIFSR_OK;
}

int sifsr_engine_forward_frozen(const float* x, float* sr, const float* params, const float* running, float* ws, size_t ws_floats,
                                int B, int H, int W, float eps, hipStream_t s) {
  if (!running || !ws) return SIFSR_ERR_ARG;
  WsLayout lay;
  SIFSR_TRY(sifsr_layout(B, H, W, 1, &lay));
  if (ws_floats < lay.total) return SIFSR_ERR_WORKSPACE;
  SIFSR_TRY(sifsr_engine_forward(x, sr, params, const_cast<float*>(running), nullptr, ws, ws_floats, B, H, W, 0, 0.f, eps, s, 0));
  return launch_bn_frozen_stats(running, eps, ws + lay.mean, ws + lay.invstd, s);
}

int sifsr_engine_backward(const float* x, const float* dsr, const float* params, float* grads, float* ws,
                          size_t ws_floats, int B, int H, int W, hipStream_t s, int bf16, int frozen, float* dx) {
  if (!x || !dsr || !params || !grads || !ws) return SIFSR_ERR_ARG;
  Ctx c{sifsr_net(), WsLayout(), ws, params, B, H, W, s};
  if (bf16 < 0 || bf16 > 1) return SIFSR_ERR_ARG;
  if ((frozen != 0 || dx != nullptr) && bf16 != 0) return SIFSR_ERR_ARG;
  c.bf16 = bf16;
  c.frozen = frozen != 0;
  const HalfStorageScope storage(bf16 == 1);
  SIFSR_TRY(sifsr_layout(B, H, W, 1, &c.lay));
  if (ws_floats < c.lay.total) return SIFSR_ERR_WORKSPACE;
  const NetTable& nt = c.nt;
  const WsLayout& w = c.lay;
  const Switches& sw = sifsr_switches();
  BwdState state;
  c.grads = grads; c.bwd = &state;
  c.side = (size_t)B * H * W >= 2u * 65536u || g_side_override == 1 ? side_lane(s) : nullptr;
  SideLaneGuard lane_guard(c.side, s);
  c.forked = &lane_guard.forked;

  const bool head_linear = sw.head_linear != 0 && dx == nullptr && bwd16_usable(c, L_IN3, src_act(c, L_IN0));
  if (head_linear) {
    hipStream_t gs = s;
    if (c.side != nullptr) {
      if (hipEventRecord(c.side->ev[L_IN0], s) != hipSuccess || hipStreamWaitEvent(c.side->s, c.side->ev[L_IN0], 0) != hipSuccess) return SIFSR_ERR_ARG;
      lane_guard.forked = true;
      gs = c.side->s;
    }
    SIFSR_TRY(launch_conv_in_gram(x, c.f(w.gram), B, H, W, gs));
    if (c.side != nullptr && hipEventRecord(c.side->aux, gs) != hipSuccess) return SIFSR_ERR_ARG;
  }
  const bool tail_in_bwd16 = !sw.tail_apply && bwd16_usable(c, L_U3B, src_act(c, L_U3A));
  {
    const LayerInfo& L = nt.L[L_U3B];
    int nblk = B * ((H + 15) / 16) * ((W + 15) / 16);
    if (nblk > 768) nblk = 768;
    SIFSR_TRY(launch_tail_bwd_reduce(c.y(L_U3B), c.scale(L_U3B), c.shift(L_U3B), c.mean(L_U3B), c.invstd(L_U3B), dsr,
                                     params + nt.out_w_off, c.f(w.slabs), c.f(w.partials), nblk, B, H, W, s, c.nf()));
    if (grads + nt.out_b_off != grads + nt.out_w_off + 144) return SIFSR_ERR_ARG;
    SIFSR_TRY(launch_bn_bwd_finalize(c.f(w.partials), nblk, 16, (double)w.npix[0], c.scale(L_U3B), c.mean(L_U3B), c.invstd(L_U3B),
                                     grads + L.gamma_off, grads + L.beta_off, c.coef(), s, c.shift(L_U3B), params + L.beta_off,
                                     c.coef_f(L_U3B), c.f(w.slabs), 145, grads + nt.out_w_off, c.frozen, c.nf()));
    if (!tail_in_bwd16)
      SIFSR_TRY(launch_tail_bwd_apply(c.y(L_U3B), c.scale(L_U3B), c.shift(L_U3B), c.coef(), dsr, params + nt.out_w_off, c.g(L_U3B),
                                      B, H, W, s));
  }

  int up_rows = 0;
  for (int k = 2; k >= 0; --k) {
    const int lv = 2 - k;
    const int la = dec_a[k], lb = dec_b[k], ls = dec_skip[k], ll = dec_low[k];
    if (k != 2) SIFSR_TRY(bn_unit_bwd(c, lb, nullptr, up_rows, 0));
    int rows_a = 0;
    SIFSR_TRY(conv_unit_bwd(c, lb, src_act(c, la), k == 2 && tail_in_bwd16 ? dsr : c.g(lb), c.g(la), nullptr, la, &rows_a,
                            k == 2 ? (tail_in_bwd16 ? 2 : 0) : 1));
    SIFSR_TRY(bn_unit_bwd(c, la, nullptr, rows_a));
    SIFSR_TRY(conv_unit_wgrad(c, la, src_raw(c.f(w.U[k]), uc[k]), src_act(c, ls), c.g(la)));
    SIFSR_TRY(conv_unit_dgrad(c, la, c.g(la), c.f(w.gU[k]), uc[k], uc[k], c.g(ls), nt.L[ls].cout, nullptr));
    up_rows = up2x_bwd_stat_rows(B, c.lvH(lv + 1), c.lvW(lv + 1), uc[k]);
    if ((size_t)up_rows * uc[k] * 2 > w.partials_cap) up_rows = 0;
    SIFSR_TRY(launch_up2x_bwd(c.f(w.gU[k]), c.g(ll), B, c.lvH(lv + 1), c.lvW(lv + 1), uc[k], s,
                              up_rows ? c.y(ll) : nullptr, up_rows ? c.scale(ll) : nullptr, up_rows ? c.shift(ll) : nullptr,
                              up_rows ? c.f(w.partials) : nullptr));
  }

  for (int k = 2; k >= 0; --k) {
    const int la = enc_a[k], lb = enc_b[k], lc = enc_c[k];
    const int er = sw.early_reduce;
    if (c.side != nullptr && (er == 3 || (er == 2 && k != 1) || (er == 1 && k == 0))) SIFSR_TRY(finish_wgrads_side(c));
    SIFSR_TRY(bn_unit_bwd(c, lc, k < 2 ? c.f(w.gP[k + 1]) : nullptr, k == 2 ? up_rows : 0, 0));
    SIFSR_TRY(conv_unit_wgrad(c, lc, src_raw(c.f(w.R[k]), pc[k]), src_none(), c.g(lc)));
    int rows_b = 0, rows_a = 0;
    SIFSR_TRY(conv_unit_dgrad(c, lc, c.g(lc), c.g(lb), pc[k], pc[k], nullptr, 0, nullptr, lb, &rows_b));
    SIFSR_TRY(bn_unit_bwd(c, lb, nullptr, rows_b));
    SIFSR_TRY(conv_unit_bwd(c, lb, src_act(c, la), c.g(lb), c.g(la), nullptr, la, &rows_a));
    SIFSR_TRY(bn_unit_bwd(c, la, nullptr, rows_a));
    SIFSR_TRY(conv_unit_bwd(c, la, src_raw(c.f(w.P[k]), pc[k]), c.g(la), c.f(w.gP[k]), c.g(lb), -1, nullptr));
  }

  const bool pool_on_load = sw.pool_on_load != 0 && bwd16_usable(c, L_IN3, src_act(c, L_IN0));
  SIFSR_TRY(bn_unit_bwd(c, L_IN3, c.f(w.gP[0]), 0, -1, !pool_on_load));
  int rows_in0 = 0;
  bool fused_in3 = false;
  SIFSR_TRY(conv_unit_bwd16(c, L_IN3, src_act(c, L_IN0), c.g(L_IN3), c.g(L_IN0), nullptr, L_IN0, &rows_in0, 1, &fused_in3, head_linear,
                            pool_on_load ? c.f(w.gP[0]) : nullptr));
  if (pool_on_load && !fused_in3) return SIFSR_ERR_ARG;
  if (head_linear && !fused_in3) return SIFSR_ERR_ARG;
  if (!fused_in3) SIFSR_TRY(conv_unit_wgrad(c, L_IN3, src_act(c, L_IN0), src_none(), c.g(L_IN3)));
  if (c.side != nullptr) SIFSR_TRY(finish_wgrads_side(c));
  if (!fused_in3) SIFSR_TRY(conv_unit_dgrad(c, L_IN3, c.g(L_IN3), c.g(L_IN0), 16, 16, nullptr, 0, nullptr, L_IN0, &rows_in0));
  {
    const LayerInfo& L = nt.L[L_IN0];
    if (rows_in0 > 0) {
      SIFSR_TRY(bn_unit_bwd(c, L_IN0, nullptr, rows_in0));
    } else {
      const size_t npix = w.npix[0];
      const int nblk_r = bn_bwd_reduce_blocks(npix);
      SIFSR_TRY(launch_bn_bwd_reduce(c.g(L_IN0), c.y(L_IN0), c.scale(L_IN0), c.shift(L_IN0), c.mean(L_IN0), c.invstd(L_IN0), 16, npix,
                                     c.f(w.partials), nblk_r, s));
      SIFSR_TRY(launch_bn_bwd_finalize(c.f(w.partials), nblk_r, 16, (double)npix, c.scale(L_IN0), c.mean(L_IN0), c.invstd(L_IN0),
                                       grads + L.gamma_off, grads + L.beta_off, c.coef(), s, nullptr, nullptr, nullptr, nullptr, 0, nullptr,
                                       c.frozen, c.nf()));
    }
    int nblk = B * ((H + 15) / 16) * ((W + 15) / 16);
    if (head_linear) {
      if (nblk > 768) nblk = 768;
      SIFSR_TRY(launch_conv_in_dz_wgrad(x, c.g(L_IN0), c.f(w.slabs), nblk, B, H, W, s));
      if (c.side != nullptr && hipStreamWaitEvent(s, c.side->aux, 0) != hipSuccess) return SIFSR_ERR_ARG;
      SIFSR_TRY(launch_conv_in_dw_combine(c.f(w.slabs), nblk, conv_in_gram_result(c.f(w.gram)), params + L.w_off, c.coef(),
                                          grads + L.w_off, s));
    } else {
      if (nblk > 1024) nblk = 1024;
      SIFSR_TRY(launch_conv_in_wgrad_fused(x, c.g(L_IN0), c.y(L_IN0), c.scale(L_IN0), c.shift(L_IN0), c.coef(), c.f(w.slabs), nblk,
                                           grads + L.w_off, B, H, W, s));
    }
    if (dx != nullptr)
      SIFSR_TRY(launch_conv_in_dgrad(c.g(L_IN0), c.y(L_IN0), c.scale(L_IN0), c.shift(L_IN0), c.coef(), params + L.w_off, dx, B, H, W, s));
  }
  if (c.side != nullptr) {
    SIFSR_TRY(lane_guard.join());
  } else {
    SIFSR_TRY(finish_wgrads(c, s));
  }
  return SIFSR_OK;
}

int sifsr_engine_set_wgrad_stream(int on) {
  g_side_override = on < 0 ? -1 : (on ? 1 : 0);
  return SIFSR_OK;
}

static int prof_add_locked(int layer, int phase) {
  if (g_prof.active >= PROF_SLOTS) return -1;
  ProfSlot& p = g_prof.slot[g_prof.active];
  while (p.start.size() < PROF_POOL) {
    hipEvent_t e0, e1;
    if (hipEventCreate(&e0) != hipSuccess) break;
    if (hipEventCreate(&e1) != hipSuccess) { (void)hipEventDestroy(e0); break; }
    p.start.push_back(e0); p.stop.push_back(e1);
  }
  p.used = 0; p.layer = layer; p.phase = phase;
  return g_prof.active++;
}
int sifsr_engine_profile_select(int layer, int phase) {
  std::lock_guard<std::mutex> lk(g_prof.mu);
  g_prof.active = 0;
  if (layer >= 0 && prof_add_locked(layer, phase) < 0) return SIFSR_ERR_ARG;
  return SIFSR_OK;
}
int sifsr_engine_profile_add(int layer, int phase) {
  if (layer < 0) return -1;
  std::lock_guard<std::mutex> lk(g_prof.mu);
  return prof_add_locked(layer, phase);
}
int sifsr_engine_profile_read(int slot, float* total_ms, int* count) {
  std::lock_guard<std::mutex> lk(g_prof.mu);
  float tot = 0.f; int n = 0;
  if (slot >= 0 && slot < g_prof.active) {
    ProfSlot& p = g_prof.slot[slot];
    for (size_t i = 0; i < p.used; ++i) {
      float ms = 0.f;
      if (hipEventSynchronize(p.stop[i]) == hipSuccess && hipEventElapsedTime(&ms, p.start[i], p.stop[i]) == hipSuccess) { tot += ms; ++n; }
    }
  }
  if (total_ms) *total_ms = tot;
  if (count) *count = n;
  return SIFSR_OK;
}
```

land-surface-temperature-super-resolution-with-a-scale-invariance-free-neural-approach_amd/csrc/loss.hip:

```cpp
#include "loss.h"

namespace {

constexpr int T = 32;
constexpr int R = 4;
constexpr int TP = T + 2 * R;
constexpr int LS = TP + 1;

__device__ __forceinline__ int refl(int i, int n) { return i < 0 ? -i : (i >= n ? 2 * (n - 1) - i : i); }
__device__ __forceinline__ float huber_val(float e) { const float a = fabsf(e); return a < 1.f ? 0.5f * e * e : a - 0.5f; }
__device__ __forceinline__ float clamp1(float e) { return e < -1.f ? -1.f : (e > 1.f ? 1.f : e); }

struct Taps { float w[9]; };
__device__ __forceinline__ float k4(int a) { return (a == 0 || a == 3) ? -0.09375f : 0.59375f; }

__device__ __forceinline__ void load_tile_reflect(float* L, const float* __restrict__ img, int H, int W, int y0,
                                                  int x0, float a, float b, int tid) {
  for (int e = tid; e < TP * TP; e += 256) {
    const int py = e / TP, px = e - py * TP;
    const int gy = refl(min(y0 - R + py, H - 1 + R), H), gx = refl(min(x0 - R + px, W - 1 + R), W);
    L[py * LS + px] = fmaf(a, img[(size_t)gy * W + gx], b);
  }
}
__device__ __forceinline__ void load_tile_zero(float* L, const float* __restrict__ img, int H, int W, int y0, int x0,
                                               int tid) {
  for (int e = tid; e < TP * TP; e += 256) {
    const int py = e / TP, px = e - py * TP;
    const int gy = y0 - R + py, gx = x0 - R + px;
    L[py * LS + px] = (gy >= 0 && gy < H && gx >= 0 && gx < W) ? img[(size_t)gy * W + gx] : 0.f;
  }
}

__device__ __forceinline__ void hpass(const float* L, float* M, const Taps& k, int tid) {
  for (int e = tid; e < TP * T; e += 256) {
    const int py = e / T, x = e - py * T;
    float s = 0.f;
#pragma unroll
    for (int t = 0; t < 9; ++t) s = fmaf(k.w[t], L[py * LS + x + t], s);
    M[py * LS + x] = s;
  }
}
__device__ __forceinline__ float vpass_at(const float* M, const Taps& k, int y, int x) {
  float s = 0.f;
#pragma unroll
  for (int t = 0; t < 9; ++t) s = fmaf(k.w[t], M[(y + t) * LS + x], s);
  return s;
}

__device__ __forceinline__ float adj_extra(const float* line, int stride, const Taps& k, int q, int g0, int n) {
  float s = 0.f;
  int u = 0;
  bool has = false;
  if (q >= 1 && q <= R) { u = -q; has = true; }
  else if (q >= n - 1 - R && q <= n - 2) { u = 2 * (n - 1) - q; has = true; }
  if (has) {
    const int lo = max(0, u - R), hi = min(n - 1, u + R);
    for (int p = lo; p <= hi; ++p) s = fmaf(k.w[u - p + R], line[(p - g0 + R) * stride], s);
  }
  return s;
}
__device__ __forceinline__ void hpass_adj(const float* V, float* M, const Taps& k, int x0, int W, int tid) {
  for (int e = tid; e < TP * T; e += 256) {
    const int py = e / T, x = e - py * T;
    float s = 0.f;
#pragma unroll
    for (int t = 0; t < 9; ++t) s = fmaf(k.w[t], V[py * LS + x + t], s);
    s += adj_extra(V + py * LS, 1, k, x0 + x, x0, W);
    M[py * LS + x] = s;
  }
}
__device__ __forceinline__ float vpass_adj_at(const float* M, const Taps& k, int y, int x, int y0, int H) {
  float s = 0.f;
#pragma unroll
  for (int t = 0; t < 9; ++t) s = fmaf(k.w[t], M[(y + t) * LS + x], s);
  s += adj_extra(M + x, LS, k, y0 + y, y0, H);
  return s;
}

__global__ __launch_bounds__(256) void blur_fwd_kernel(const float* __restrict__ x, float* __restrict__ out, Taps k,
                                                       int H, int W) {
  __shared__ float L[TP * LS], M[TP * LS];
  const int tid = threadIdx.x, x0 = blockIdx.x * T, y0 = blockIdx.y * T;
  const size_t img = (size_t)blockIdx.z * H * W;
  load_tile_reflect(L, x + img, H, W, y0, x0, 1.f, 0.f, tid);
  __syncthreads();
  hpass(L, M, k, tid);
  __syncthreads();
  const int tx = tid & 31, ty = tid >> 5;
#pragma unroll
  for (int r = 0; r < 4; ++r) {
    const int y = ty + 8 * r;
    if (y0 + y < H && x0 + tx < W) out[img + (size_t)(y0 + y) * W + x0 + tx] = vpass_at(M, k, y, tx);
  }
}

__global__ __launch_bounds__(256) void blur_bwd_kernel(const float* __restrict__ g, float* __restrict__ out, Taps k,
                                                       int H, int W) {
  __shared__ float L[TP * LS], M[TP * LS];
  const int tid = threadIdx.x, x0 = blockIdx.x * T, y0 = blockIdx.y * T;
  const size_t img = (size_t)blockIdx.z * H * W;
  load_tile_zero(L, g + img, H, W, y0, x0, tid);
  __syncthreads();
  hpass_adj(L, M, k, x0, W, tid);
  __syncthreads();
  const int tx = tid & 31, ty = tid >> 5;
#pragma unroll
  for (int r = 0; r < 4; ++r) {
    const int y = ty + 8 * r;
    if (y0 + y < H && x0 + tx < W) out[img + (size_t)(y0 + y) * W + x0 + tx] = vpass_adj_at(M, k, y, tx, y0, H);
  }
}

__global__ __launch_bounds__(256) void blurdec_fwd_kernel(const float* __restrict__ x, float* __restrict__ out, Taps k,
                                                          int H, int W) {
  __shared__ float L[TP * LS], M[TP * LS];
  const int tid = threadIdx.x, x0 = blockIdx.x * T, y0 = blockIdx.y * T;
  const size_t img = (size_t)blockIdx.z * H * W;
  load_tile_reflect(L, x + img, H, W, y0, x0, 1.f, 0.f, tid);
  __syncthreads();
  hpass(L, M, k, tid);
  __syncthreads();
  const int tx = tid & 31, ty = tid >> 5;
  float* Bt = L;
  float v[4];
#pragma unroll
  for (int r = 0; r < 4; ++r) v[r] = vpass_at(M, k, ty + 8 * r, tx);
  __syncthreads();
#pragma unroll
  for (int r = 0; r < 4; ++r) Bt[(ty + 8 * r) * LS + tx] = v[r];
  __syncthreads();
  if (tid < 64) {
    const int i = tid >> 3, j = tid & 7;
    float s = 0.f;
#pragma unroll
    for (int a = 0; a < 4; ++a)
#pragma unroll
      for (int b = 0; b < 4; ++b) s = fmaf(k4(a) * k4(b), Bt[(4 * i + a) * LS + 4 * j + b], s);
    if (y0 / 4 + i < H / 4 && x0 / 4 + j < W / 4)
      out[(size_t)blockIdx.z * (H / 4) * (W / 4) + (size_t)(y0 / 4 + i) * (W / 4) + x0 / 4 + j] = s;
  }
}

__device__ __forceinline__ void load_tile_dect(float* L, const float* __restrict__ glr, int H, int W, int y0, int x0,
                                               int tid) {
  for (int e = tid; e < TP * TP; e += 256) {
    const int py = e / TP, px = e - py * TP;
    const int gy = y0 - R + py, gx = x0 - R + px;
    L[py * LS + px] = (gy >= 0 && gy < H && gx >= 0 && gx < W)
                          ? k4(gy & 3) * k4(gx & 3) * glr[(size_t)(gy >> 2) * (W / 4) + (gx >> 2)] : 0.f;
  }
}

__global__ __launch_bounds__(256) void blurdec_bwd_kernel(const float* __restrict__ glr, float* __restrict__ out,
                                                          Taps k, int H, int W) {
  __shared__ float L[TP * LS], M[TP * LS];
  const int tid = threadIdx.x, x0 = blockIdx.x * T, y0 = blockIdx.y * T;
  load_tile_dect(L, glr + (size_t)blockIdx.z * (H / 4) * (W / 4), H, W, y0, x0, tid);
  __syncthreads();
  hpass_adj(L, M, k, x0, W, tid);
  __syncthreads();
  const int tx = tid & 31, ty = tid >> 5;
  const size_t img = (size_t)blockIdx.z * H * W;
#pragma unroll
  for (int r = 0; r < 4; ++r) {
    const int y = ty + 8 * r;
    if (y0 + y < H && x0 + tx < W) out[img + (size_t)(y0 + y) * W + x0 + tx] = vpass_adj_at(M, k, y, tx, y0, H);
  }
}

__device__ __forceinline__ void sobel4(const float n[9], float o[4]) {
  o[0] = (n[0] + 2.f * n[1] + n[2]) - (n[6] + 2.f * n[7] + n[8]);
  o[1] = (n[0] + 2.f * n[3] + n[6]) - (n[2] + 2.f * n[5] + n[8]);
  o[2] = (2.f * n[0] + n[1] + n[3]) - (n[5] + n[7] + 2.f * n[8]);
  o[3] = (n[1] + 2.f * n[2] + n[5]) - (n[3] + 2.f * n[6] + n[7]);
}
__device__ __forceinline__ void neigh9_zero(const float* __restrict__ img, int H, int W, int y, int x, float n[9]) {
#pragma unroll
  for (int t = 0; t < 9; ++t) {
    const int yy = y + t / 3 - 1, xx = x + t % 3 - 1;
    n[t] = (yy >= 0 && yy < H && xx >= 0 && xx < W) ? img[(size_t)yy * W + xx] : 0.f;
  }
}

__global__ void sobel_fwd_kernel(const float* __restrict__ x, float* __restrict__ out, int B, int H, int W) {
  const size_t n = (size_t)B * H * W;
  for (size_t e = (size_t)blockIdx.x * blockDim.x + threadIdx.x; e < n; e += (size_t)gridDim.x * blockDim.x) {
    const int xx = e % W, yy = (e / W) % H;
    const size_t b = e / ((size_t)W * H);
    float nb[9], o[4];
    neigh9_zero(x + b * H * W, H, W, yy, xx, nb);
    sobel4(nb, o);
#pragma unroll
    for (int f = 0; f < 4; ++f) out[((b * 4 + f) * H + yy) * W + xx] = o[f];
  }
}

__device__ __forceinline__ float sobel_adj_at(const float* __restrict__ g, size_t plane, int H, int W, int y, int x) {
  const float F[4][9] = {{1, 2, 1, 0, 0, 0, -1, -2, -1}, {1, 0, -1, 2, 0, -2, 1, 0, -1},
                         {2, 1, 0, 1, 0, -1, 0, -1, -2}, {0, 1, 2, -1, 0, 1, -2, -1, 0}};
  float s = 0.f;
#pragma unroll
  for (int t = 0; t < 9; ++t) {
    const int yy = y - (t / 3 - 1), xx = x - (t % 3 - 1);
    if (yy >= 0 && yy < H && xx >= 0 && xx < W) {
#pragma unroll
      for (int f = 0; f < 4; ++f)
        if (F[f][t] != 0.f) s = fmaf(F[f][t], g[f * plane + (size_t)yy * W + xx], s);
    }
  }
  return s;
}

__global__ void sobel_bwd_kernel(const float* __restrict__ g, float* __restrict__ out, int B, int H, int W) {
  const size_t n = (size_t)B * H * W, plane = (size_t)H * W;
  for (size_t e = (size_t)blockIdx.x * blockDim.x + threadIdx.x; e < n; e += (size_t)gridDim.x * blockDim.x) {
    const int xx = e % W, yy = (e / W) % H;
    const size_t b = e / plane;
    out[e] = sobel_adj_at(g + b * 4 * plane, plane, H, W, yy, xx);
  }
}

__device__ __forceinline__ float block_sum(float v, float* sh) {
#pragma unroll
  for (int m = 1; m < 64; m <<= 1) v += __shfl_xor(v, m);
  const int tid = threadIdx.x;
  if ((tid & 63) == 0) sh[tid >> 6] = v;
  __syncthreads();
  v = sh[0] + sh[1] + sh[2] + sh[3];
  __syncthreads();
  return v;
}

__global__ __launch_bounds__(256) void huber_partial_kernel(const float* __restrict__ a, const float* __restrict__ b,
                                                            float bscale, size_t n, float* __restrict__ partials) {
  __shared__ float sh[4];
  float s = 0.f;
  for (size_t e = (size_t)blockIdx.x * 256 + threadIdx.x; e < n; e += (size_t)gridDim.x * 256)
    s += huber_val(a[e] - bscale * b[e]);
  s = block_sum(s, sh);
  if (threadIdx.x == 0) partials[blockIdx.x] = s;
}

__device__ __forceinline__ void masked_scales(const long long* __restrict__ n_valid, double per_lr, float* sc0, float* sc1) {
  const long long n = n_valid[0];
  const double n1 = (double)n, n2 = per_lr * (double)n;
  *sc0 = n > 0 ? (float)(1.0 / n1) : 0.f;
  *sc1 = n > 0 ? (float)(1.0 / n2) : 0.f;
}

__global__ __launch_bounds__(256) void loss_finalize_kernel(const float* __restrict__ partials, int nblk, int stride,
                                                            int nout, float sc0, float sc1, float alpha,
                                                            float* __restrict__ out, const long long* __restrict__ n_valid,
                                                            double per_lr) {
  __shared__ double r[2][256];
  const int tid = threadIdx.x;
  if (n_valid != nullptr) masked_scales(n_valid, per_lr, &sc0, &sc1);
  double s0 = 0.0, s1 = 0.0;
  for (int k = tid; k < nblk; k += 256) {
    s0 += (double)partials[(size_t)k * stride];
    if (nout > 1) s1 += (double)partials[(size_t)k * stride + 1];
  }
  r[0][tid] = s0; r[1][tid] = s1;
  __syncthreads();
  for (int st = 128; st > 0; st >>= 1) {
    if (tid < st) { r[0][tid] += r[0][tid + st]; r[1][tid] += r[1][tid + st]; }
    __syncthreads();
  }
  if (tid == 0) {
    const float l0 = (float)(r[0][0] * (double)sc0);
    out[0] = l0;
    if (nout > 1) {
      const float l1 = (float)(r[1][0] * (double)sc1);
      out[1] = l1;
      out[2] = alpha * l0 + (1.f - alpha) * l1;
    }
  }
}

__global__ void huber_bwd_kernel(const float* __restrict__ a, const float* __restrict__ b, float bscale,
                                 const float* __restrict__ gout, float inv_n, size_t n, float* __restrict__ ga) {
  const float go = gout[0] * inv_n;
  for (size_t e = (size_t)blockIdx.x * blockDim.x + threadIdx.x; e < n; e += (size_t)gridDim.x * blockDim.x)
    ga[e] = go * clamp1(a[e] - bscale * b[e]);
}

template <int KIND, bool MASKED>
__global__ __launch_bounds__(256) void sif_loss_fwd_kernel(const float* __restrict__ sr, const float* __restrict__ lst,
                                                           const float* __restrict__ ndvi, Taps k1, Taps k2, float mean,
                                                           float std, float gamma, float w1, float w2,
                                                           float* __restrict__ r1, float* __restrict__ r2,
                                                           float* __restrict__ partials, int H, int W,
                                                           const unsigned char* __restrict__ valid,
                                                           const long long* __restrict__ n_valid, float alpha) {
  __shared__ float L[TP * LS], M[TP * LS], N[TP * LS];
  __shared__ float sh[4];
  __shared__ unsigned char vt[64];
  if constexpr (MASKED) {
    const long long n = n_valid[0];
    const double n1 = (double)n, n2 = (KIND == 1 ? 64.0 : 16.0) * (double)n;
    w1 = n > 0 ? (float)((double)alpha / n1) : 0.f;
    w2 = n > 0 ? (float)((1.0 - (double)alpha) / n2) : 0.f;
  }
  const int tid = threadIdx.x, x0 = blockIdx.x * T, y0 = blockIdx.y * T;
  const int tx = tid & 31, ty = tid >> 5;
  const size_t img = (size_t)blockIdx.z * H * W;
  const size_t blk = ((size_t)blockIdx.z * gridDim.y + blockIdx.y) * gridDim.x + blockIdx.x;
  float h1 = 0.f, h2 = 0.f;

  load_tile_reflect(L, sr + img, H, W, y0, x0, std, mean, tid);
  __syncthreads();
  hpass(L, M, k1, tid);
  __syncthreads();
  {
    float v[4];
#pragma unroll
    for (int r = 0; r < 4; ++r) v[r] = vpass_at(M, k1, ty + 8 * r, tx);
#pragma unroll
    for (int r = 0; r < 4; ++r) N[(ty + 8 * r) * LS + tx] = v[r];
  }
  __syncthreads();
  if (tid < 64) {
    const int i = tid >> 3, j = tid & 7;
    float s = 0.f;
#pragma unroll
    for (int a = 0; a < 4; ++a)
#pragma unroll
      for (int b = 0; b < 4; ++b) s = fmaf(k4(a) * k4(b), N[(4 * i + a) * LS + 4 * j + b], s);
    bool ok = true;
    if (y0 / 4 + i < H / 4 && x0 / 4 + j < W / 4) {
      const size_t o = (size_t)blockIdx.z * (H / 4) * (W / 4) + (size_t)(y0 / 4 + i) * (W / 4) + x0 / 4 + j;
      if constexpr (MASKED) ok = valid[o] != 0;
      if (ok) {
        const float e = (s - mean) / std - lst[o];
        h1 = huber_val(e);
        r1[o] = w1 * clamp1(e);
      } else {
        r1[o] = 0.f;
      }
    } else {
      ok = false;
    }
    if constexpr (MASKED) vt[tid] = ok ? 1 : 0;
  }
  __syncthreads();

  if (KIND == 2) {
    load_tile_reflect(L, sr + img, H, W, y0, x0, 1.f, 0.f, tid);
    __syncthreads();
    hpass(L, M, k2, tid);
    __syncthreads();
    float hs[4];
#pragma unroll
    for (int r = 0; r < 4; ++r) hs[r] = L[(ty + 8 * r + R) * LS + tx + R] - vpass_at(M, k2, ty + 8 * r, tx);
    __syncthreads();
    load_tile_reflect(L, ndvi + img, H, W, y0, x0, 1.f, 0.f, tid);
    __syncthreads();
    hpass(L, M, k2, tid);
    __syncthreads();
#pragma unroll
    for (int r = 0; r < 4; ++r) {
      const int y = ty + 8 * r;
      const float hn = L[(y + R) * LS + tx + R] - vpass_at(M, k2, y, tx);
      const float e = hs[r] - gamma * hn;
      if (y0 + y < H && x0 + tx < W) {
        float hv = huber_val(e), rv = w2 * clamp1(e);
        if constexpr (MASKED) {
          if (vt[(y >> 2) * 8 + (tx >> 2)] == 0) hv = rv = 0.f;
        }
        h2 += hv;
        r2[img + (size_t)(y0 + y) * W + x0 + tx] = rv;
      }
    }
  } else {
#pragma unroll
    for (int r = 0; r < 4; ++r) {
      const int y = y0 + ty + 8 * r, x = x0 + tx;
      if (y >= H || x >= W) continue;
      if constexpr (MASKED) {
        if (vt[((ty + 8 * r) >> 2) * 8 + (tx >> 2)] == 0) {
          st4(r2 + (img + (size_t)y * W + x) * 4, make_float4(0.f, 0.f, 0.f, 0.f));
          continue;
        }
      }
      float nb[9], a[4], c[4];
      neigh9_zero(sr + img, H, W, y, x, nb);
      sobel4(nb, a);
      neigh9_zero(ndvi + img, H, W, y, x, nb);
      sobel4(nb, c);
      float4 o;
      float e;
      e = a[0] - gamma * c[0]; h2 += huber_val(e); o.x = w2 * clamp1(e);
      e = a[1] - gamma * c[1]; h2 += huber_val(e); o.y = w2 * clamp1(e);
      e = a[2] - gamma * c[2]; h2 += huber_val(e); o.z = w2 * clamp1(e);
      e = a[3] - gamma * c[3]; h2 += huber_val(e); o.w = w2 * clamp1(e);
      st4(r2 + (img + (size_t)y * W + x) * 4, o);
    }
  }
  h1 = block_sum(h1, sh);
  h2 = block_sum(h2, sh);
  if (tid == 0) { partials[blk * 2] = h1; partials[blk * 2 + 1] = h2; }
}

template <int KIND, bool MASKED>
__global__ __launch_bounds__(256) void sif_loss_bwd_kernel(const float* __restrict__ r1, const float* __restrict__ r2,
                                                           Taps k1, Taps k2, float* __restrict__ dsr, int H, int W,
                                                           const float* __restrict__ fin_partials, int fin_nblk, float fin_sc0,
                                                           float fin_sc1, float fin_alpha, float* __restrict__ fin_out,
                                                           const long long* __restrict__ n_valid) {
  __shared__ float L[TP * LS], M[TP * LS];
  __shared__ double fin_w[4][2];
  const int tid = threadIdx.x, x0 = blockIdx.x * T, y0 = blockIdx.y * T;
  const int tx = tid & 31, ty = tid >> 5;
  const size_t img = (size_t)blockIdx.z * H * W;
  float acc[4];
  load_tile_dect(L, r1 + (size_t)blockIdx.z * (H / 4) * (W / 4), H, W, y0, x0, tid);
  __syncthreads();
  hpass_adj(L, M, k1, x0, W, tid);
  __syncthreads();
#pragma unroll
  for (int r = 0; r < 4; ++r) acc[r] = vpass_adj_at(M, k1, ty + 8 * r, tx, y0, H);
  __syncthreads();
  if (KIND == 2) {
    load_tile_zero(L, r2 + img, H, W, y0, x0, tid);
    __syncthreads();
    hpass_adj(L, M, k2, x0, W, tid);
    __syncthreads();
#pragma unroll
    for (int r = 0; r < 4; ++r) {
      const int y = ty + 8 * r;
      acc[r] += L[(y + R) * LS + tx + R] - vpass_adj_at(M, k2, y, tx, y0, H);
    }
  } else {
    const float F[4][9] = {{1, 2, 1, 0, 0, 0, -1, -2, -1}, {1, 0, -1, 2, 0, -2, 1, 0, -1},
                           {2, 1, 0, 1, 0, -1, 0, -1, -2}, {0, 1, 2, -1, 0, 1, -2, -1, 0}};
#pragma unroll
    for (int r = 0; r < 4; ++r) {
      const int y = y0 + ty + 8 * r, x = x0 + tx;
      float s = 0.f;
#pragma unroll
      for (int t = 0; t < 9; ++t) {
        const int yy = y - (t / 3 - 1), xx = x - (t % 3 - 1);
        if (y < H && x < W && yy >= 0 && yy < H && xx >= 0 && xx < W) {
          const float4 g = ld4(r2 + (img + (size_t)yy * W + xx) * 4);
          s += F[0][t] * g.x + F[1][t] * g.y + F[2][t] * g.z + F[3][t] * g.w;
        }
      }
      acc[r] += s;
    }
  }
#pragma unroll
  for (int r = 0; r < 4; ++r)
    if (y0 + ty + 8 * r < H && x0 + tx < W) dsr[img + (size_t)(y0 + ty + 8 * r) * W + x0 + tx] = acc[r];
  if (fin_out != nullptr && blockIdx.x == 0 && blockIdx.y == 0 && blockIdx.z == 0) {
    if constexpr (MASKED) masked_scales(n_valid, KIND == 1 ? 64.0 : 16.0, &fin_sc0, &fin_sc1);
    double s0 = 0.0, s1 = 0.0;
    for (int k = tid; k < fin_nblk; k += 256) { s0 += (double)fin_partials[2 * (size_t)k]; s1 += (double)fin_partials[2 * (size_t)k + 1]; }
#pragma unroll
    for (int m = 32; m > 0; m >>= 1) { s0 += __shfl_xor(s0, m); s1 += __shfl_xor(s1, m); }
    if ((tid & 63) == 0) { fin_w[tid >> 6][0] = s0; fin_w[tid >> 6][1] = s1; }
    __syncthreads();
    if (tid == 0) {
      const float l0 = (float)((fin_w[0][0] + fin_w[1][0] + fin_w[2][0] + fin_w[3][0]) * (double)fin_sc0);
      const float l1 = (float)((fin_w[0][1] + fin_w[1][1] + fin_w[2][1] + fin_w[3][1]) * (double)fin_sc1);
      fin_out[0] = l0; fin_out[1] = l1;
      fin_out[2] = fin_alpha * l0 + (1.f - fin_alpha) * l1;
    }
  }
}

inline Taps make_taps(const float* t9) { Taps k; for (int i = 0; i < 9; ++i) k.w[i] = t9[i]; return k; }
inline int ew_grid(size_t n) { size_t b = (n + 255) / 256; return (int)(b > 8192 ? 8192 : (b < 1 ? 1 : b)); }

}


#define SIFSR_CHECK_ANY(H, W, M) if ((H) < 2 * R + 2 || (W) < 2 * R + 2 || (H) % (M) || (W) % (M) || B < 1 || B > 65535) return SIFSR_ERR_SHAPE
#define SIFSR_TGRID(H, W, B) dim3(((W) + T - 1) / T, ((H) + T - 1) / T, B)

int launch_blur_fwd(const float* x, const float* taps9, float* out, int B, int H, int W, hipStream_t s) {
  SIFSR_CHECK_ANY(H, W, 1);
  hipLaunchKernelGGL(blur_fwd_kernel, SIFSR_TGRID(H, W, B), dim3(256), 0, s, x, out, make_taps(taps9), H, W);
  SIFSR_LAUNCH_CHECK();
  return SIFSR_OK;
}
int launch_blur_bwd(const float* g, const float* taps9, float* out, int B, int H, int W, hipStream_t s) {
  SIFSR_CHECK_ANY(H, W, 1);
  hipLaunchKernelGGL(blur_bwd_kernel, SIFSR_TGRID(H, W, B), dim3(256), 0, s, g, out, make_taps(taps9), H, W);
  SIFSR_LAUNCH_CHECK();
  return SIFSR_OK;
}
int launch_blurdec_fwd(const float* x, const float* taps9, float* out, int B, int H, int W, hipStream_t s) {
  SIFSR_CHECK_ANY(H, W, 4);
  hipLaunchKernelGGL(blurdec_fwd_kernel, SIFSR_TGRID(H, W, B), dim3(256), 0, s, x, out, make_taps(taps9), H, W);
  SIFSR_LAUNCH_CHECK();
  return SIFSR_OK;
}
int launch_blurdec_bwd(const float* glr, const float* taps9, float* out, int B, int H, int W, hipStream_t s) {
  SIFSR_CHECK_ANY(H, W, 4);
  hipLaunchKernelGGL(blurdec_bwd_kernel, SIFSR_TGRID(H, W, B), dim3(256), 0, s, glr, out, make_taps(taps9), H, W);
  SIFSR_LAUNCH_CHECK();
  return SIFSR_OK;
}
int launch_sobel_fwd(const float* x, float* out, int B, int H, int W, hipStream_t s) {
  hipLaunchKernelGGL(sobel_fwd_kernel, dim3(ew_grid((size_t)B * H * W)), dim3(256), 0, s, x, out, B, H, W);
  SIFSR_LAUNCH_CHECK();
  return SIFSR_OK;
}
int launch_sobel_bwd(const float* g, float* out, int B, int H, int W, hipStream_t s) {
  hipLaunchKernelGGL(sobel_bwd_kernel, dim3(ew_grid((size_t)B * H * W)), dim3(256), 0, s, g, out, B, H, W);
  SIFSR_LAUNCH_CHECK();
  return SIFSR_OK;
}
int huber_partial_blocks(size_t n) { size_t b = (n + 4095) / 4096; return (int)(b > 1024 ? 1024 : (b < 1 ? 1 : b)); }
int launch_huber_fwd(const float* a, const float* b, float bscale, size_t n, float* partials, float* out, hipStream_t s) {
  const int nblk = huber_partial_blocks(n);
  hipLaunchKernelGGL(huber_partial_kernel, dim3(nblk), dim3(256), 0, s, a, b, bscale, n, partials);
  hipLaunchKernelGGL(loss_finalize_kernel, dim3(1), dim3(256), 0, s, partials, nblk, 1, 1, (float)(1.0 / (double)n), 0.f, 0.f, out, (const long long*)nullptr, 0.0);
  SIFSR_LAUNCH_CHECK();
  return SIFSR_OK;
}
int launch_huber_bwd(const float* a, const float* b, float bscale, const float* gout, size_t n, float* ga, hipStream_t s) {
  hipLaunchKernelGGL(huber_bwd_kernel, dim3(ew_grid(n)), dim3(256), 0, s, a, b, bscale, gout, (float)(1.0 / (double)n), n, ga);
  SIFSR_LAUNCH_CHECK();
  return SIFSR_OK;
}

size_t sif_loss_workspace_floats(int kind, int B, int H, int W) {
  const size_t hr = (size_t)B * H * W, lr = hr / 16, nblk = (size_t)B * ((H + T - 1) / T) * ((W + T - 1) / T);
  return lr + (kind == 1 ? 4 * hr : hr) + 2 * nblk;
}

namespace {

template <int KIND, bool MASKED>
void sif_loss_launch(const float* sr, const float* lst, const unsigned char* valid, const long long* n_valid, const float* ndvi,
                     int B, int H, int W, float mean, float std, float alpha, float gamma, const Taps& k1, const Taps& k2,
                     float* ws, float* losses3, float* dsr, hipStream_t s) {
  const size_t hr = (size_t)B * H * W, lr = hr / 16;
  const int nblk = B * ((H + T - 1) / T) * ((W + T - 1) / T);
  float* r1 = ws;
  float* r2 = r1 + lr;
  float* partials = r2 + (KIND == 1 ? 4 * hr : hr);
  const double n1 = (double)lr, n2 = KIND == 1 ? 4.0 * (double)hr : (double)hr;
  const float w1 = (float)((double)alpha / n1), w2 = (float)((1.0 - (double)alpha) / n2);
  const dim3 grid = SIFSR_TGRID(H, W, B);
  hipLaunchKernelGGL((sif_loss_fwd_kernel<KIND, MASKED>), grid, dim3(256), 0, s, sr, lst, ndvi, k1, k2, mean, std, gamma, w1, w2, r1,
                     r2, partials, H, W, valid, n_valid, alpha);
  if (dsr != nullptr)
    hipLaunchKernelGGL((sif_loss_bwd_kernel<KIND, MASKED>), grid, dim3(256), 0, s, r1, r2, k1, k2, dsr, H, W, partials, nblk,
                       (float)(1.0 / n1), (float)(1.0 / n2), alpha, losses3, n_valid);
  else
    hipLaunchKernelGGL(loss_finalize_kernel, dim3(1), dim3(256), 0, s, partials, nblk, 2, 2, (float)(1.0 / n1), (float)(1.0 / n2),
                       alpha, losses3, n_valid, KIND == 1 ? 64.0 : 16.0);
}

}

int launch_sif_loss(int kind, const float* sr, const float* lst, const float* ndvi, int B, int H, int W, float mean,
                    float std, float alpha, float gamma, const float* taps_ds, const float* taps_ftm, float* ws,
                    float* losses3, float* dsr, hipStream_t s) {
  SIFSR_CHECK_ANY(H, W, 4);
  if (kind != 1 && kind != 2) return SIFSR_ERR_ARG;
  const Taps k1 = make_taps(taps_ds), k2 = make_taps(taps_ftm);
  if (kind == 2) sif_loss_launch<2, false>(sr, lst, nullptr, nullptr, ndvi, B, H, W, mean, std, alpha, gamma, k1, k2, ws, losses3, dsr, s);
  else sif_loss_launch<1, false>(sr, lst, nullptr, nullptr, ndvi, B, H, W, mean, std, alpha, gamma, k1, k2, ws, losses3, dsr, s);
  SIFSR_LAUNCH_CHECK();
  return SIFSR_OK;
}

int launch_sif_loss_masked(int kind, const float* sr, const float* lst, const unsigned char* valid, const long long* n_valid,
                           const float* ndvi, int B, int H, int W, float mean, float std, float alpha, float gamma,
                           const float* taps_ds, const float* taps_ftm, float* ws, float* losses3, float* dsr, hipStream_t s) {
  SIFSR_CHECK_ANY(H, W, 4);
  if (kind != 1 && kind != 2) return SIFSR_ERR_ARG;
  const Taps k1 = make_taps(taps_ds), k2 = make_taps(taps_ftm);
  if (kind == 2) sif_loss_launch<2, true>(sr, lst, valid, n_valid, ndvi, B, H, W, mean, std, alpha, gamma, k1, k2, ws, losses3, dsr, s);
  else sif_loss_launch<1, true>(sr, lst, valid, n_valid, ndvi, B, H, W, mean, std, alpha, gamma, k1, k2, ws, losses3, dsr, s);
  SIFSR_LAUNCH_CHECK();
  return SIFSR_OK;
}
```

Measured before the change: 10710 patches/s.

## Recompute conv_in output in wgrad, prefetch tiles, vectorize loss blur passes

New measurement: 10770 patches/s (median of 6 runs). Within noise of the previous version (+0.6%).

```diff
diff --git a/land-surface-temperature-super-resolution-with-a-scale-invariance-free-neural-approach_amd/csrc/edge_conv.h b/land-surface-temperature-super-resolution-with-a-scale-invariance-free-neural-approach_amd/csrc/edge_conv.h
--- a/land-surface-temperature-super-resolution-with-a-scale-invariance-free-neural-approach_amd/csrc/edge_conv.h
+++ b/land-surface-temperature-super-resolution-with-a-scale-invariance-free-neural-approach_amd/csrc/edge_conv.h
@@ -12,7 +12,8 @@
 int launch_conv_out_wgrad(const float* y, const float* scale, const float* shift, const float* dsr, float* partials,
                           int nblk, float* dw, float* db, int B, int H, int W, hipStream_t s);
 int launch_conv_in_wgrad_fused(const float* x, const float* g, const float* y, const float* scale, const float* shift,
-                               const double* coef, float* partials, int nblk, float* dw, int B, int H, int W, hipStream_t s);
+                               const double* coef, float* partials, int nblk, float* dw, int B, int H, int W, hipStream_t s,
+                               const float* w0 = nullptr);
 size_t conv_in_gram_scratch_floats();
 int launch_conv_in_gram(const float* x, float* scratch, int B, int H, int W, hipStream_t s);
 const double* conv_in_gram_result(const float* scratch);
diff --git a/land-surface-temperature-super-resolution-with-a-scale-invariance-free-neural-approach_amd/csrc/edge_conv.hip b/land-surface-temperature-super-resolution-with-a-scale-invariance-free-neural-approach_amd/csrc/edge_conv.hip
--- a/land-surface-temperature-super-resolution-with-a-scale-invariance-free-neural-approach_amd/csrc/edge_conv.hip
+++ b/land-surface-temperature-super-resolution-with-a-scale-invariance-free-neural-approach_amd/csrc/edge_conv.hip
@@ -1,6 +1,22 @@
 #include "edge_conv.h"
 
 namespace {
+
+static __device__ __forceinline__ void conv_in_operands(const float* __restrict__ w, int i, int kq, float (&wa)[5], int (&off)[5]) {
+#pragma unroll
+  for (int j = 0; j < 5; ++j) {
+    const int kk = 4 * j + kq;
+    wa[j] = kk < 18 ? w[i * 18 + kk] : 0.f;
+    const int c = kk >= 9 ? 1 : 0, t = kk < 18 ? kk - 9 * c : 0;
+    off[j] = (kk < 18 ? c * 324 : 0) + (t / 3) * 18 + t % 3 + i;
+  }
+}
+static __device__ __forceinline__ f32x4 conv_in_row(const float (&wa)[5], const int (&off)[5], const float* T, int row) {
+  f32x4 acc = (f32x4){0.f, 0.f, 0.f, 0.f};
+#pragma unroll
+  for (int j = 0; j < 5; ++j) acc = __builtin_amdgcn_mfma_f32_16x16x4f32(wa[j], T[off[j] + row * 18], acc, 0, 0, 0);
+  return acc;
+}
 
 template <bool HS>
 __global__ __launch_bounds__(256) void conv_in_fwd_kernel(const float* __restrict__ x, const float* __restrict__ w,
@@ -24,13 +40,7 @@
   if ((int)blockIdx.x < ntiles) stage(blockIdx.x, tile[0]);
   float wa[5];
   int off[5];
-#pragma unroll
-  for (int j = 0; j < 5; ++j) {
-    const int kk = 4 * j + kq;
-    wa[j] = kk < 18 ? w[i * 18 + kk] : 0.f;
-    const int c = kk >= 9 ? 1 : 0, t = kk < 18 ? kk - 9 * c : 0;
-    off[j] = (kk < 18 ? c * 324 : 0) + (t / 3) * 18 + t % 3 + i;
-  }
+  conv_in_operands(w, i, kq, wa, off);
   float s1[4] = {0.f, 0.f, 0.f, 0.f}, s2[4] = {0.f, 0.f, 0.f, 0.f};
   int buf = 0;
   for (int t = blockIdx.x; t < ntiles; t += gridDim.x, buf ^= 1) {
@@ -43,9 +53,7 @@
 #pragma unroll
     for (int r = 0; r < 4; ++r) {
       const int row = 4 * wave + r;
-      f32x4 acc = (f32x4){0.f, 0.f, 0.f, 0.f};
-#pragma unroll
-      for (int j = 0; j < 5; ++j) acc = __builtin_amdgcn_mfma_f32_16x16x4f32(wa[j], T[off[j] + row * 18], acc, 0, 0, 0);
+      const f32x4 acc = conv_in_row(wa, off, T, row);
       if (y0 + row < H && x0 + i < W) {
         const float4 o = as_stored4<HS>(make_float4(acc[0], acc[1], acc[2], acc[3]));
         stA4<HS>(y, ((size_t)(b * H + y0 + row) * W + x0 + i) * 16 + 4 * kq, o);
@@ -72,15 +80,16 @@
   }
 }
 
-template <bool FUSED, bool HS>
+template <bool FUSED, bool HS, bool RECOMPUTE>
 __global__ __launch_bounds__(256) void conv_in_wgrad_kernel(const float* __restrict__ x, const float* __restrict__ dy,
-                                                            const float* __restrict__ yraw,
+                                                            const float* __restrict__ yraw, const float* __restrict__ w0,
                                                             const float* __restrict__ scale,
                                                             const float* __restrict__ shift,
                                                             const double* __restrict__ coef,
                                                             float* __restrict__ partials, int B, int H, int W) {
+  static_assert(!RECOMPUTE || (FUSED && !HS), "RECOMPUTE rebuilds the fp32 y of the fused form; a bf16-stored y is read");
   SIFSR_CHAIN_PRIO();
-  __shared__ float tile[2 * 324 + 8];
+  __shared__ float tile[2][2 * 324 + 8];
   __shared__ float dyt[256 * 16];
   __shared__ float red[4][2][256];
   const int tid = threadIdx.x, lane = tid & 63, wave = tid >> 6;
@@ -96,46 +105,77 @@
   float4 sc4, sh4;
   double sd[4], k1[4], k0[4];
   if (FUSED) {
-    const int q4 = tid & 3;
-    sc4 = ld4(scale + 4 * q4); sh4 = ld4(shift + 4 * q4);
-#pragma unroll
-    for (int j = 0; j < 4; ++j) { sd[j] = coef[4 * q4 + j]; k1[j] = coef[16 + 4 * q4 + j]; k0[j] = coef[32 + 4 * q4 + j]; }
-  }
-  for (int tl = blockIdx.x; tl < ntiles; tl += gridDim.x) {
+    sc4 = ld4(scale + 4 * k); sh4 = ld4(shift + 4 * k);
+#pragma unroll
+    for (int j = 0; j < 4; ++j) { sd[j] = coef[4 * k + j]; k1[j] = coef[16 + 4 * k + j]; k0[j] = coef[32 + 4 * k + j]; }
+  }
+  float wa[5];
+  int off[5];
+  if constexpr (RECOMPUTE) conv_in_operands(w0, i16, k, wa, off);
+  int hc[3], hy[3], hx[3];
+#pragma unroll
+  for (int j = 0; j < 3; ++j) {
+    const int e = min(tid + 256 * j, 2 * 324 - 1);
+    hc[j] = e / 324;
+    hy[j] = (e - hc[j] * 324) / 18;
+    hx[j] = e - hc[j] * 324 - hy[j] * 18;
+  }
+  float ph[3];
+  float4 pg[4], py[4];
+  bool pin[4];
+  auto fetch = [&](int tl) __attribute__((always_inline)) {
     const int tx = tl % tiles_x, ty = (tl / tiles_x) % tiles_y, b = tl / (tiles_x * tiles_y);
     const int x0 = tx * 16, y0 = ty * 16;
-    __syncthreads();
-    for (int e = tid; e < 2 * 324; e += 256) {
-      const int c = e / 324, p = e - c * 324;
-      const int py = p / 18, px = p - py * 18;
-      const int gy = clampi(y0 - 1 + py, 0, H - 1), gx = clampi(x0 - 1 + px, 0, W - 1);
-      tile[e] = x[((size_t)(b * 2 + c) * H + gy) * W + gx];
-    }
-    for (int e = tid; e < 256 * 4; e += 256) {
-      const int p = e >> 2, c4 = e & 3;
-      if (y0 + (p >> 4) >= H || x0 + (p & 15) >= W) {
-        *reinterpret_cast<float4*>(&dyt[p * 16 + 4 * c4]) = make_float4(0.f, 0.f, 0.f, 0.f);
-        continue;
-      }
-      const size_t off = ((size_t)(b * H + y0 + (p >> 4)) * W + x0 + (p & 15)) * 16 + 4 * c4;
-      float4 v = ldA4<HS>(dy, off);
+#pragma unroll
+    for (int j = 0; j < 3; ++j)
+      ph[j] = x[((size_t)(b * 2 + hc[j]) * H + clampi(y0 - 1 + hy[j], 0, H - 1)) * W + clampi(x0 - 1 + hx[j], 0, W - 1)];
+    const int gx = min(x0 + i16, W - 1);
+#pragma unroll
+    for (int r = 0; r < 4; ++r) {
+      const int gy = y0 + 4 * wave + r;
+      pin[r] = gy < H && x0 + i16 < W;
+      const size_t o = ((size_t)(b * H + min(gy, H - 1)) * W + gx) * 16 + 4 * k;
+      pg[r] = ldA4<HS>(dy, o);
+      if constexpr (FUSED && !RECOMPUTE) py[r] = ldA4<HS>(yraw, o);
+    }
+  };
+  if ((int)blockIdx.x < ntiles) fetch(blockIdx.x);
+  int buf = 0;
+  for (int tl = blockIdx.x; tl < ntiles; tl += gridDim.x, buf ^= 1) {
+    float* T = tile[buf];
+    T[tid] = ph[0];
+    T[tid + 256] = ph[1];
+    if (tid + 512 < 2 * 324) T[tid + 512] = ph[2];
+    __syncthreads();
+#pragma unroll
+    for (int r = 0; r < 4; ++r) {
+      const int row = 4 * wave + r;
+      float4 v = pg[r];
       if (FUSED) {
-        const float4 yv = ldA4<HS>(yraw, off);
+        float4 yv;
+        if constexpr (RECOMPUTE) {
+          const f32x4 a = conv_in_row(wa, off, T, row);
+          yv = make_float4(a[0], a[1], a[2], a[3]);
+        } else {
+          yv = py[r];
+        }
         v.x = (float)fma(sd[0], (double)(fmaf(yv.x, sc4.x, sh4.x) > 0.f ? v.x : 0.f), fma(k1[0], (double)yv.x, k0[0]));
         v.y = (float)fma(sd[1], (double)(fmaf(yv.y, sc4.y, sh4.y) > 0.f ? v.y : 0.f), fma(k1[1], (double)yv.y, k0[1]));
         v.z = (float)fma(sd[2], (double)(fmaf(yv.z, sc4.z, sh4.z) > 0.f ? v.z : 0.f), fma(k1[2], (double)yv.z, k0[2]));
         v.w = (float)fma(sd[3], (double)(fmaf(yv.w, sc4.w, sh4.w) > 0.f ? v.w : 0.f), fma(k1[3], (double)yv.w, k0[3]));
       }
-      *reinterpret_cast<float4*>(&dyt[p * 16 + 4 * c4]) = v;
-    }
-    __syncthreads();
+      if (!pin[r]) v = make_float4(0.f, 0.f, 0.f, 0.f);
+      *reinterpret_cast<float4*>(&dyt[(row * 16 + i16) * 16 + 4 * k]) = v;
+    }
+    __syncthreads();
+    if (tl + (int)gridDim.x < ntiles) fetch(tl + gridDim.x);
 #pragma unroll 4
     for (int ks = wave; ks < 64; ks += 4) {
       const int r = ks >> 2, qd = ks & 3;
       const float av = dyt[(r * 16 + 4 * qd + k) * 16 + i16];
       const int base = r * 18 + 4 * qd + k;
-      acc[0] = __builtin_amdgcn_mfma_f32_16x16x4f32(av, tile[offn[0] + base], acc[0], 0, 0, 0);
-      acc[1] = __builtin_amdgcn_mfma_f32_16x16x4f32(av, tile[offn[1] + base], acc[1], 0, 0, 0);
+      acc[0] = __builtin_amdgcn_mfma_f32_16x16x4f32(av, T[offn[0] + base], acc[0], 0, 0, 0);
+      acc[1] = __builtin_amdgcn_mfma_f32_16x16x4f32(av, T[offn[1] + base], acc[1], 0, 0, 0);
     }
   }
 #pragma unroll
@@ -549,8 +589,8 @@
 int launch_conv_in_wgrad(const float* x, const float* dy, float* partials, int nblk, float* dw, int B, int H, int W,
                          hipStream_t s) {
   if (H < 1 || W < 1) return SIFSR_ERR_SHAPE;
-  if (sifsr_half_storage()) hipLaunchKernelGGL((conv_in_wgrad_kernel<false, true>), dim3(nblk), dim3(256), 0, s, x, dy, nullptr, nullptr, nullptr, nullptr, partials, B, H, W);
-  else hipLaunchKernelGGL((conv_in_wgrad_kernel<false, false>), dim3(nblk), dim3(256), 0, s, x, dy, nullptr, nullptr, nullptr, nullptr, partials, B, H, W);
+  if (sifsr_half_storage()) hipLaunchKernelGGL((conv_in_wgrad_kernel<false, true, false>), dim3(nblk), dim3(256), 0, s, x, dy, nullptr, nullptr, nullptr, nullptr, nullptr, partials, B, H, W);
+  else hipLaunchKernelGGL((conv_in_wgrad_kernel<false, false, false>), dim3(nblk), dim3(256), 0, s, x, dy, nullptr, nullptr, nullptr, nullptr, nullptr, partials, B, H, W);
   hipLaunchKernelGGL(sum_partials_kernel, dim3(72), dim3(256), 0, s, partials, nblk, 288, dw);
   SIFSR_LAUNCH_CHECK();
   return SIFSR_OK;
@@ -558,10 +598,12 @@
 
 int launch_conv_in_wgrad_fused(const float* x, const float* g, const float* y, const float* scale, const float* shift,
                                const double* coef, float* partials, int nblk, float* dw, int B, int H, int W,
-                               hipStream_t s) {
+                               hipStream_t s, const float* w0) {
   if (H < 1 || W < 1) return SIFSR_ERR_SHAPE;
-  if (sifsr_half_storage()) hipLaunchKernelGGL((conv_in_wgrad_kernel<true, true>), dim3(nblk), dim3(256), 0, s, x, g, y, scale, shift, coef, partials, B, H, W);
-  else hipLaunchKernelGGL((conv_in_wgrad_kernel<true, false>), dim3(nblk), dim3(256), 0, s, x, g, y, scale, shift, coef, partials, B, H, W);
+  if (w0 != nullptr && sifsr_half_storage()) return SIFSR_ERR_ARG;
+  if (sifsr_half_storage()) hipLaunchKernelGGL((conv_in_wgrad_kernel<true, true, false>), dim3(nblk), dim3(256), 0, s, x, g, y, nullptr, scale, shift, coef, partials, B, H, W);
+  else if (w0 != nullptr) hipLaunchKernelGGL((conv_in_wgrad_kernel<true, false, true>), dim3(nblk), dim3(256), 0, s, x, g, nullptr, w0, scale, shift, coef, partials, B, H, W);
+  else hipLaunchKernelGGL((conv_in_wgrad_kernel<true, false, false>), dim3(nblk), dim3(256), 0, s, x, g, y, nullptr, scale, shift, coef, partials, B, H, W);
   hipLaunchKernelGGL(sum_partials_kernel, dim3(72), dim3(256), 0, s, partials, nblk, 288, dw);
   SIFSR_LAUNCH_CHECK();
   return SIFSR_OK;
diff --git a/land-surface-temperature-super-resolution-with-a-scale-invariance-free-neural-approach_amd/csrc/engine.hip b/land-surface-temperature-super-resolution-with-a-scale-invariance-free-neural-approach_amd/csrc/engine.hip
--- a/land-surface-temperature-super-resolution-with-a-scale-invariance-free-neural-approach_amd/csrc/engine.hip
+++ b/land-surface-temperature-super-resolution-with-a-scale-invariance-free-neural-approach_amd/csrc/engine.hip
@@ -642,8 +642,9 @@
                                           grads + L.w_off, s));
     } else {
       if (nblk > 1024) nblk = 1024;
+      const float* w0 = c.bf16 == 0 ? params + L.w_off : nullptr;
       SIFSR_TRY(launch_conv_in_wgrad_fused(x, c.g(L_IN0), c.y(L_IN0), c.scale(L_IN0), c.shift(L_IN0), c.coef(), c.f(w.slabs), nblk,
-                                           grads + L.w_off, B, H, W, s));
+                                           grads + L.w_off, B, H, W, s, w0));
     }
     if (dx != nullptr)
       SIFSR_TRY(launch_conv_in_dgrad(c.g(L_IN0), c.y(L_IN0), c.scale(L_IN0), c.shift(L_IN0), c.coef(), params + L.w_off, dx, B, H, W, s));
diff --git a/land-surface-temperature-super-resolution-with-a-scale-invariance-free-neural-approach_amd/csrc/loss.hip b/land-surface-temperature-super-resolution-with-a-scale-invariance-free-neural-approach_amd/csrc/loss.hip
--- a/land-surface-temperature-super-resolution-with-a-scale-invariance-free-neural-approach_amd/csrc/loss.hip
+++ b/land-surface-temperature-super-resolution-with-a-scale-invariance-free-neural-approach_amd/csrc/loss.hip
@@ -1,3 +1,5 @@
+#include <cstdint>
+
 #include "loss.h"
 
 namespace {
@@ -5,7 +7,9 @@
 constexpr int T = 32;
 constexpr int R = 4;
 constexpr int TP = T + 2 * R;
-constexpr int LS = TP + 1;
+constexpr int TQ = TP / 4;
+constexpr int LS = TP + 4;
+constexpr int MS = T + 4;
 
 __device__ __forceinline__ int refl(int i, int n) { return i < 0 ? -i : (i >= n ? 2 * (n - 1) - i : i); }
 __device__ __forceinline__ float huber_val(float e) { const float a = fabsf(e); return a < 1.f ? 0.5f * e * e : a - 0.5f; }
@@ -14,37 +18,61 @@
 struct Taps { float w[9]; };
 __device__ __forceinline__ float k4(int a) { return (a == 0 || a == 3) ? -0.09375f : 0.59375f; }
 
-__device__ __forceinline__ void load_tile_reflect(float* L, const float* __restrict__ img, int H, int W, int y0,
-                                                  int x0, float a, float b, int tid) {
-  for (int e = tid; e < TP * TP; e += 256) {
-    const int py = e / TP, px = e - py * TP;
-    const int gy = refl(min(y0 - R + py, H - 1 + R), H), gx = refl(min(x0 - R + px, W - 1 + R), W);
-    L[py * LS + px] = fmaf(a, img[(size_t)gy * W + gx], b);
-  }
-}
-__device__ __forceinline__ void load_tile_zero(float* L, const float* __restrict__ img, int H, int W, int y0, int x0,
-                                               int tid) {
-  for (int e = tid; e < TP * TP; e += 256) {
-    const int py = e / TP, px = e - py * TP;
-    const int gy = y0 - R + py, gx = x0 - R + px;
-    L[py * LS + px] = (gy >= 0 && gy < H && gx >= 0 && gx < W) ? img[(size_t)gy * W + gx] : 0.f;
-  }
-}
-
-__device__ __forceinline__ void hpass(const float* L, float* M, const Taps& k, int tid) {
-  for (int e = tid; e < TP * T; e += 256) {
-    const int py = e / T, x = e - py * T;
-    float s = 0.f;
-#pragma unroll
-    for (int t = 0; t < 9; ++t) s = fmaf(k.w[t], L[py * LS + x + t], s);
-    M[py * LS + x] = s;
-  }
-}
-__device__ __forceinline__ float vpass_at(const float* M, const Taps& k, int y, int x) {
-  float s = 0.f;
-#pragma unroll
-  for (int t = 0; t < 9; ++t) s = fmaf(k.w[t], M[(y + t) * LS + x], s);
-  return s;
+__device__ __forceinline__ bool aligned16(const float* p) { return (reinterpret_cast<uintptr_t>(p) & 15) == 0; }
+__device__ __forceinline__ void st4v(float* p, const float v[4]) { st4(p, make_float4(v[0], v[1], v[2], v[3])); }
+
+enum TileMode { REFLECT, ZERO, DECT };
+template <TileMode MODE>
+__device__ __forceinline__ void tile_quad(const float* __restrict__ img, int H, int W, int yy, int xx, bool rowvec, float (&v)[4]) {
+  if constexpr (MODE == REFLECT) {
+    const float* row = img + (size_t)refl(min(yy, H - 1 + R), H) * W;
+    if (rowvec) {
+      const float4 g = ld4(row + xx);
+      v[0] = g.x; v[1] = g.y; v[2] = g.z; v[3] = g.w;
+    } else {
+#pragma unroll
+      for (int j = 0; j < 4; ++j) v[j] = row[refl(min(xx + j, W - 1 + R), W)];
+    }
+  } else if constexpr (MODE == ZERO) {
+    const bool in = yy >= 0 && yy < H;
+    const float* row = img + (size_t)(in ? yy : 0) * W;
+    if (in && rowvec) {
+      const float4 g = ld4(row + xx);
+      v[0] = g.x; v[1] = g.y; v[2] = g.z; v[3] = g.w;
+    } else {
+#pragma unroll
+      for (int j = 0; j < 4; ++j) v[j] = (in && xx + j >= 0 && xx + j < W) ? row[xx + j] : 0.f;
+    }
+  } else {
+    const bool in = yy >= 0 && yy < H && xx >= 0 && xx < W;
+    const float g = in ? img[(size_t)(yy >> 2) * (W / 4) + (xx >> 2)] : 0.f;
+#pragma unroll
+    for (int j = 0; j < 4; ++j) v[j] = in ? k4(yy & 3) * k4(j) * g : 0.f;
+  }
+}
+template <TileMode MODE, int N>
+__device__ __forceinline__ void load_tiles(float* const (&L)[N], const float* const (&img)[N], int H, int W, int y0, int x0, int tid) {
+  bool rowvec = MODE != DECT && x0 >= R && x0 + T + R <= W && (W & 3) == 0;
+#pragma unroll
+  for (int n = 0; n < N; ++n) rowvec = rowvec && aligned16(img[n]);
+  constexpr int NIT = (TP * TQ + 255) / 256;
+  float v[NIT][N][4];
+#pragma unroll
+  for (int it = 0; it < NIT; ++it) {
+    const int e = tid + 256 * it, py = e / TQ, c = e - py * TQ;
+    if (e < TP * TQ) {
+#pragma unroll
+      for (int n = 0; n < N; ++n) tile_quad<MODE>(img[n], H, W, y0 - R + py, x0 - R + 4 * c, rowvec, v[it][n]);
+    }
+  }
+#pragma unroll
+  for (int it = 0; it < NIT; ++it) {
+    const int e = tid + 256 * it, py = e / TQ, c = e - py * TQ;
+    if (e < TP * TQ) {
+#pragma unroll
+      for (int n = 0; n < N; ++n) st4v(L[n] + py * LS + 4 * c, v[it][n]);
+    }
+  }
 }
 
 __device__ __forceinline__ float adj_extra(const float* line, int stride, const Taps& k, int q, int g0, int n) {
@@ -59,112 +87,102 @@
   }
   return s;
 }
-__device__ __forceinline__ void hpass_adj(const float* V, float* M, const Taps& k, int x0, int W, int tid) {
-  for (int e = tid; e < TP * T; e += 256) {
-    const int py = e / T, x = e - py * T;
-    float s = 0.f;
-#pragma unroll
-    for (int t = 0; t < 9; ++t) s = fmaf(k.w[t], V[py * LS + x + t], s);
-    s += adj_extra(V + py * LS, 1, k, x0 + x, x0, W);
-    M[py * LS + x] = s;
-  }
-}
-__device__ __forceinline__ float vpass_adj_at(const float* M, const Taps& k, int y, int x, int y0, int H) {
+
+template <bool ADJ>
+__device__ __forceinline__ void hpass(const float* L, float* M, const Taps& k, float a, float b, int x0, int W, int tid) {
+  for (int e = tid; e < TP * (T / 4); e += 256) {
+    const int q = e / TP, py = e - q * TP;
+    const float* row = L + py * LS;
+    const float4 i0 = ld4(row + 4 * q), i1 = ld4(row + 4 * q + 4), i2 = ld4(row + 4 * q + 8);
+    float in[12] = {i0.x, i0.y, i0.z, i0.w, i1.x, i1.y, i1.z, i1.w, i2.x, i2.y, i2.z, i2.w};
+    if constexpr (!ADJ) {
+#pragma unroll
+      for (int i = 0; i < 12; ++i) in[i] = fmaf(a, in[i], b);
+    }
+    float o[4];
+#pragma unroll
+    for (int j = 0; j < 4; ++j) {
+      float s = 0.f;
+#pragma unroll
+      for (int t = 0; t < 9; ++t) s = fmaf(k.w[t], in[j + t], s);
+      if constexpr (ADJ) s += adj_extra(row, 1, k, x0 + 4 * q + j, x0, W);
+      o[j] = s;
+    }
+    st4v(M + py * MS + 4 * q, o);
+  }
+}
+template <bool ADJ>
+__device__ __forceinline__ void vpass(const float* M, const Taps& k, int y, int q, int y0, int H, float o[4]) {
+  float s[4] = {0.f, 0.f, 0.f, 0.f};
+#pragma unroll
+  for (int t = 0; t < 9; ++t) {
+    const float4 m = ld4(M + (y + t) * MS + 4 * q);
+    s[0] = fmaf(k.w[t], m.x, s[0]); s[1] = fmaf(k.w[t], m.y, s[1]);
+    s[2] = fmaf(k.w[t], m.z, s[2]); s[3] = fmaf(k.w[t], m.w, s[3]);
+  }
+#pragma unroll
+  for (int j = 0; j < 4; ++j) {
+    if constexpr (ADJ) s[j] += adj_extra(M + 4 * q + j, MS, k, y0 + y, y0, H);
+    o[j] = s[j];
+  }
+}
+
+__device__ __forceinline__ void store_quad(float* row, int x, int W, const float v[4], bool vec) {
+  if (vec) {
+    if (x < W) st4v(row + x, v);
+  } else {
+#pragma unroll
+    for (int j = 0; j < 4; ++j)
+      if (x + j < W) row[x + j] = v[j];
+  }
+}
+
+__device__ __forceinline__ float decimate_at(const float* Bt, int i, int j) {
   float s = 0.f;
 #pragma unroll
-  for (int t = 0; t < 9; ++t) s = fmaf(k.w[t], M[(y + t) * LS + x], s);
-  s += adj_extra(M + x, LS, k, y0 + y, y0, H);
+  for (int a = 0; a < 4; ++a) {
+    const float4 d = ld4(Bt + (4 * i + a) * MS + 4 * j);
+    s = fmaf(k4(a) * k4(0), d.x, s); s = fmaf(k4(a) * k4(1), d.y, s);
+    s = fmaf(k4(a) * k4(2), d.z, s); s = fmaf(k4(a) * k4(3), d.w, s);
+  }
   return s;
 }
 
-__global__ __launch_bounds__(256) void blur_fwd_kernel(const float* __restrict__ x, float* __restrict__ out, Taps k,
-                                                       int H, int W) {
-  __shared__ float L[TP * LS], M[TP * LS];
+template <TileMode MODE>
+__global__ __launch_bounds__(256) void blur_kernel(const float* __restrict__ g, float* __restrict__ out, Taps k, int H, int W) {
+  __shared__ __align__(16) float L[TP * LS], M[TP * MS];
+  constexpr bool ADJ = MODE != REFLECT;
   const int tid = threadIdx.x, x0 = blockIdx.x * T, y0 = blockIdx.y * T;
+  const int vy = tid & 31, vq = tid >> 5;
   const size_t img = (size_t)blockIdx.z * H * W;
-  load_tile_reflect(L, x + img, H, W, y0, x0, 1.f, 0.f, tid);
-  __syncthreads();
-  hpass(L, M, k, tid);
-  __syncthreads();
-  const int tx = tid & 31, ty = tid >> 5;
-#pragma unroll
-  for (int r = 0; r < 4; ++r) {
-    const int y = ty + 8 * r;
-    if (y0 + y < H && x0 + tx < W) out[img + (size_t)(y0 + y) * W + x0 + tx] = vpass_at(M, k, y, tx);
-  }
-}
-
-__global__ __launch_bounds__(256) void blur_bwd_kernel(const float* __restrict__ g, float* __restrict__ out, Taps k,
-                                                       int H, int W) {
-  __shared__ float L[TP * LS], M[TP * LS];
-  const int tid = threadIdx.x, x0 = blockIdx.x * T, y0 = blockIdx.y * T;
-  const size_t img = (size_t)blockIdx.z * H * W;
-  load_tile_zero(L, g + img, H, W, y0, x0, tid);
-  __syncthreads();
-  hpass_adj(L, M, k, x0, W, tid);
-  __syncthreads();
-  const int tx = tid & 31, ty = tid >> 5;
-#pragma unroll
-  for (int r = 0; r < 4; ++r) {
-    const int y = ty + 8 * r;
-    if (y0 + y < H && x0 + tx < W) out[img + (size_t)(y0 + y) * W + x0 + tx] = vpass_adj_at(M, k, y, tx, y0, H);
-  }
+  load_tiles<MODE, 1>({L}, {g + (MODE == DECT ? (size_t)blockIdx.z * (H / 4) * (W / 4) : img)}, H, W, y0, x0, tid);
+  __syncthreads();
+  hpass<ADJ>(L, M, k, 1.f, 0.f, x0, W, tid);
+  __syncthreads();
+  float v[4];
+  vpass<ADJ>(M, k, vy, vq, y0, H, v);
+  if (y0 + vy < H) store_quad(out + img + (size_t)(y0 + vy) * W, x0 + 4 * vq, W, v, (W & 3) == 0 && aligned16(out + img));
 }
 
 __global__ __launch_bounds__(256) void blurdec_fwd_kernel(const float* __restrict__ x, float* __restrict__ out, Taps k,
                                                           int H, int W) {
-  __shared__ float L[TP * LS], M[TP * LS];
+  __shared__ __align__(16) float L[TP * LS], M[TP * MS], Bt[T * MS];
   const int tid = threadIdx.x, x0 = blockIdx.x * T, y0 = blockIdx.y * T;
+  const int vy = tid & 31, vq = tid >> 5;
   const size_t img = (size_t)blockIdx.z * H * W;
-  load_tile_reflect(L, x + img, H, W, y0, x0, 1.f, 0.f, tid);
-  __syncthreads();
-  hpass(L, M, k, tid);
-  __syncthreads();
-  const int tx = tid & 31, ty = tid >> 5;
-  float* Bt = L;
+  load_tiles<REFLECT, 1>({L}, {x + img}, H, W, y0, x0, tid);
+  __syncthreads();
+  hpass<false>(L, M, k, 1.f, 0.f, x0, W, tid);
+  __syncthreads();
   float v[4];
-#pragma unroll
-  for (int r = 0; r < 4; ++r) v[r] = vpass_at(M, k, ty + 8 * r, tx);
-  __syncthreads();
-#pragma unroll
-  for (int r = 0; r < 4; ++r) Bt[(ty + 8 * r) * LS + tx] = v[r];
+  vpass<false>(M, k, vy, vq, y0, H, v);
+  st4v(Bt + vy * MS + 4 * vq, v);
   __syncthreads();
   if (tid < 64) {
     const int i = tid >> 3, j = tid & 7;
-    float s = 0.f;
-#pragma unroll
-    for (int a = 0; a < 4; ++a)
-#pragma unroll
-      for (int b = 0; b < 4; ++b) s = fmaf(k4(a) * k4(b), Bt[(4 * i + a) * LS + 4 * j + b], s);
+    const float s = decimate_at(Bt, i, j);
     if (y0 / 4 + i < H / 4 && x0 / 4 + j < W / 4)
       out[(size_t)blockIdx.z * (H / 4) * (W / 4) + (size_t)(y0 / 4 + i) * (W / 4) + x0 / 4 + j] = s;
-  }
-}
-
-__device__ __forceinline__ void load_tile_dect(float* L, const float* __restrict__ glr, int H, int W, int y0, int x0,
-                                               int tid) {
-  for (int e = tid; e < TP * TP; e += 256) {
-    const int py = e / TP, px = e - py * TP;
-    const int gy = y0 - R + py, gx = x0 - R + px;
-    L[py * LS + px] = (gy >= 0 && gy < H && gx >= 0 && gx < W)
-                          ? k4(gy & 3) * k4(gx & 3) * glr[(size_t)(gy >> 2) * (W / 4) + (gx >> 2)] : 0.f;
-  }
-}
-
-__global__ __launch_bounds__(256) void blurdec_bwd_kernel(const float* __restrict__ glr, float* __restrict__ out,
-                                                          Taps k, int H, int W) {
-  __shared__ float L[TP * LS], M[TP * LS];
-  const int tid = threadIdx.x, x0 = blockIdx.x * T, y0 = blockIdx.y * T;
-  load_tile_dect(L, glr + (size_t)blockIdx.z * (H / 4) * (W / 4), H, W, y0, x0, tid);
-  __syncthreads();
-  hpass_adj(L, M, k, x0, W, tid);
-  __syncthreads();
-  const int tx = tid & 31, ty = tid >> 5;
-  const size_t img = (size_t)blockIdx.z * H * W;
-#pragma unroll
-  for (int r = 0; r < 4; ++r) {
-    const int y = ty + 8 * r;
-    if (y0 + y < H && x0 + tx < W) out[img + (size_t)(y0 + y) * W + x0 + tx] = vpass_adj_at(M, k, y, tx, y0, H);
   }
 }
 
@@ -220,25 +238,28 @@
   }
 }
 
-__device__ __forceinline__ float block_sum(float v, float* sh) {
-#pragma unroll
-  for (int m = 1; m < 64; m <<= 1) v += __shfl_xor(v, m);
+template <int NV>
+__device__ __forceinline__ void block_sum(float (&v)[NV], float* sh) {
   const int tid = threadIdx.x;
-  if ((tid & 63) == 0) sh[tid >> 6] = v;
-  __syncthreads();
-  v = sh[0] + sh[1] + sh[2] + sh[3];
-  __syncthreads();
-  return v;
+#pragma unroll
+  for (int i = 0; i < NV; ++i) {
+#pragma unroll
+    for (int m = 1; m < 64; m <<= 1) v[i] += __shfl_xor(v[i], m);
+    if ((tid & 63) == 0) sh[4 * i + (tid >> 6)] = v[i];
+  }
+  __syncthreads();
+#pragma unroll
+  for (int i = 0; i < NV; ++i) v[i] = sh[4 * i] + sh[4 * i + 1] + sh[4 * i + 2] + sh[4 * i + 3];
 }
 
 __global__ __launch_bounds__(256) void huber_partial_kernel(const float* __restrict__ a, const float* __restrict__ b,
                                                             float bscale, size_t n, float* __restrict__ partials) {
   __shared__ float sh[4];
-  float s = 0.f;
+  float s[1] = {0.f};
   for (size_t e = (size_t)blockIdx.x * 256 + threadIdx.x; e < n; e += (size_t)gridDim.x * 256)
-    s += huber_val(a[e] - bscale * b[e]);
-  s = block_sum(s, sh);
-  if (threadIdx.x == 0) partials[blockIdx.x] = s;
+    s[0] += huber_val(a[e] - bscale * b[e]);
+  block_sum(s, sh);
+  if (threadIdx.x == 0) partials[blockIdx.x] = s[0];
 }
 
 __device__ __forceinline__ void masked_scales(const long long* __restrict__ n_valid, double per_lr, float* sc0, float* sc1) {
@@ -285,15 +306,17 @@
 }
 
 template <int KIND, bool MASKED>
-__global__ __launch_bounds__(256) void sif_loss_fwd_kernel(const float* __restrict__ sr, const float* __restrict__ lst,
+__global__ __launch_bounds__(256, 7) void sif_loss_fwd_kernel(const float* __restrict__ sr, const float* __restrict__ lst,
                                                            const float* __restrict__ ndvi, Taps k1, Taps k2, float mean,
                                                            float std, float gamma, float w1, float w2,
                                                            float* __restrict__ r1, float* __restrict__ r2,
                                                            float* __restrict__ partials, int H, int W,
                                                            const unsigned char* __restrict__ valid,
                                                            const long long* __restrict__ n_valid, float alpha) {
-  __shared__ float L[TP * LS], M[TP * LS], N[TP * LS];
-  __shared__ float sh[4];
+  constexpr bool HF = KIND == 2;
+  __shared__ __align__(16) float S[TP * LS], M[TP * MS], Bt[T * MS];
+  float* const HV = Bt;
+  __shared__ float sh[8];
   __shared__ unsigned char vt[64];
   if constexpr (MASKED) {
     const long long n = n_valid[0];
@@ -302,75 +325,74 @@
     w2 = n > 0 ? (float)((1.0 - (double)alpha) / n2) : 0.f;
   }
   const int tid = threadIdx.x, x0 = blockIdx.x * T, y0 = blockIdx.y * T;
+  const int vy = tid & 31, vq = tid >> 5;
   const int tx = tid & 31, ty = tid >> 5;
   const size_t img = (size_t)blockIdx.z * H * W;
   const size_t blk = ((size_t)blockIdx.z * gridDim.y + blockIdx.y) * gridDim.x + blockIdx.x;
-  float h1 = 0.f, h2 = 0.f;
-
-  load_tile_reflect(L, sr + img, H, W, y0, x0, std, mean, tid);
-  __syncthreads();
-  hpass(L, M, k1, tid);
+  const int li = tid >> 3, lj = tid & 7;
+  const bool lr_in = tid < 64 && y0 / 4 + li < H / 4 && x0 / 4 + lj < W / 4;
+  const size_t lo = (size_t)blockIdx.z * (H / 4) * (W / 4) + (size_t)(y0 / 4 + li) * (W / 4) + x0 / 4 + lj;
+  bool lr_ok = lr_in;
+  if constexpr (MASKED) {
+    if (lr_in) lr_ok = valid[lo] != 0;
+    if (tid < 64) vt[tid] = lr_ok ? 1 : 0;
+  }
+  float h[2] = {0.f, 0.f};
+
+  load_tiles<REFLECT, 1>({S}, {sr + img}, H, W, y0, x0, tid);
+  __syncthreads();
+  hpass<false>(S, M, k1, std, mean, x0, W, tid);
   __syncthreads();
   {
     float v[4];
-#pragma unroll
-    for (int r = 0; r < 4; ++r) v[r] = vpass_at(M, k1, ty + 8 * r, tx);
-#pragma unroll
-    for (int r = 0; r < 4; ++r) N[(ty + 8 * r) * LS + tx] = v[r];
+    vpass<false>(M, k1, vy, vq, y0, H, v);
+    st4v(Bt + vy * MS + 4 * vq, v);
   }
   __syncthreads();
   if (tid < 64) {
-    const int i = tid >> 3, j = tid & 7;
-    float s = 0.f;
-#pragma unroll
-    for (int a = 0; a < 4; ++a)
-#pragma unroll
-      for (int b = 0; b < 4; ++b) s = fmaf(k4(a) * k4(b), N[(4 * i + a) * LS + 4 * j + b], s);
-    bool ok = true;
-    if (y0 / 4 + i < H / 4 && x0 / 4 + j < W / 4) {
-      const size_t o = (size_t)blockIdx.z * (H / 4) * (W / 4) + (size_t)(y0 / 4 + i) * (W / 4) + x0 / 4 + j;
-      if constexpr (MASKED) ok = valid[o] != 0;
-      if (ok) {
-        const float e = (s - mean) / std - lst[o];
-        h1 = huber_val(e);
-        r1[o] = w1 * clamp1(e);
-      } else {
-        r1[o] = 0.f;
-      }
-    } else {
-      ok = false;
-    }
-    if constexpr (MASKED) vt[tid] = ok ? 1 : 0;
-  }
-  __syncthreads();
-
-  if (KIND == 2) {
-    load_tile_reflect(L, sr + img, H, W, y0, x0, 1.f, 0.f, tid);
-    __syncthreads();
-    hpass(L, M, k2, tid);
-    __syncthreads();
-    float hs[4];
-#pragma unroll
-    for (int r = 0; r < 4; ++r) hs[r] = L[(ty + 8 * r + R) * LS + tx + R] - vpass_at(M, k2, ty + 8 * r, tx);
-    __syncthreads();
-    load_tile_reflect(L, ndvi + img, H, W, y0, x0, 1.f, 0.f, tid);
-    __syncthreads();
-    hpass(L, M, k2, tid);
-    __syncthreads();
-#pragma unroll
-    for (int r = 0; r < 4; ++r) {
-      const int y = ty + 8 * r;
-      const float hn = L[(y + R) * LS + tx + R] - vpass_at(M, k2, y, tx);
-      const float e = hs[r] - gamma * hn;
-      if (y0 + y < H && x0 + tx < W) {
-        float hv = huber_val(e), rv = w2 * clamp1(e);
-        if constexpr (MASKED) {
-          if (vt[(y >> 2) * 8 + (tx >> 2)] == 0) hv = rv = 0.f;
-        }
-        h2 += hv;
-        r2[img + (size_t)(y0 + y) * W + x0 + tx] = rv;
-      }
-    }
+    const float s = decimate_at(Bt, li, lj);
+    if (lr_ok) {
+      const float e = (s - mean) / std - lst[lo];
+      h[0] = huber_val(e);
+      r1[lo] = w1 * clamp1(e);
+    } else if (lr_in) {
+      r1[lo] = 0.f;
+    }
+  }
+  if constexpr (HF) {
+    float hs[4], g[4];
+    hpass<false>(S, M, k2, 1.f, 0.f, x0, W, tid);
+    __syncthreads();
+    vpass<false>(M, k2, vy, vq, y0, H, g);
+    float4 c = ld4(S + (vy + R) * LS + 4 * vq + R);
+    hs[0] = fmaf(1.f, c.x, 0.f) - g[0]; hs[1] = fmaf(1.f, c.y, 0.f) - g[1];
+    hs[2] = fmaf(1.f, c.z, 0.f) - g[2]; hs[3] = fmaf(1.f, c.w, 0.f) - g[3];
+    __syncthreads();
+    load_tiles<REFLECT, 1>({S}, {ndvi + img}, H, W, y0, x0, tid);
+    __syncthreads();
+    hpass<false>(S, M, k2, 1.f, 0.f, x0, W, tid);
+    __syncthreads();
+    vpass<false>(M, k2, vy, vq, y0, H, g);
+    c = ld4(S + (vy + R) * LS + 4 * vq + R);
+    const float cn[4] = {fmaf(1.f, c.x, 0.f), fmaf(1.f, c.y, 0.f), fmaf(1.f, c.z, 0.f), fmaf(1.f, c.w, 0.f)};
+    const bool in = y0 + vy < H && x0 + 4 * vq < W;
+    bool ok = in;
+    if constexpr (MASKED) ok = in && vt[(vy >> 2) * 8 + vq] != 0;
+    float hv[4], rv[4];
+#pragma unroll
+    for (int j = 0; j < 4; ++j) {
+      const float hn = cn[j] - g[j];
+      const float e = hs[j] - gamma * hn;
+      hv[j] = ok ? huber_val(e) : 0.f;
+      rv[j] = ok ? w2 * clamp1(e) : 0.f;
+    }
+    st4v(HV + vy * MS + 4 * vq, hv);
+    if (in) store_quad(r2 + img + (size_t)(y0 + vy) * W, x0 + 4 * vq, W, rv, aligned16(r2 + img));
+    __syncthreads();
+  }
+  if constexpr (HF) {
+#pragma unroll
+    for (int r = 0; r < 4; ++r) h[1] += HV[(ty + 8 * r) * MS + tx];
   } else {
 #pragma unroll
     for (int r = 0; r < 4; ++r) {
@@ -389,16 +411,15 @@
       sobel4(nb, c);
       float4 o;
       float e;
-      e = a[0] - gamma * c[0]; h2 += huber_val(e); o.x = w2 * clamp1(e);
-      e = a[1] - gamma * c[1]; h2 += huber_val(e); o.y = w2 * clamp1(e);
-      e = a[2] - gamma * c[2]; h2 += huber_val(e); o.z = w2 * clamp1(e);
-      e = a[3] - gamma * c[3]; h2 += huber_val(e); o.w = w2 * clamp1(e);
+      e = a[0] - gamma * c[0]; h[1] += huber_val(e); o.x = w2 * clamp1(e);
+      e = a[1] - gamma * c[1]; h[1] += huber_val(e); o.y = w2 * clamp1(e);
+      e = a[2] - gamma * c[2]; h[1] += huber_val(e); o.z = w2 * clamp1(e);
+      e = a[3] - gamma * c[3]; h[1] += huber_val(e); o.w = w2 * clamp1(e);
       st4(r2 + (img + (size_t)y * W + x) * 4, o);
     }
   }
-  h1 = block_sum(h1, sh);
-  h2 = block_sum(h2, sh);
-  if (tid == 0) { partials[blk * 2] = h1; partials[blk * 2 + 1] = h2; }
+  block_sum(h, sh);
+  if (tid == 0) { partials[blk * 2] = h[0]; partials[blk * 2 + 1] = h[1]; }
 }
 
 template <int KIND, bool MASKED>
@@ -407,35 +428,31 @@
                                                            const float* __restrict__ fin_partials, int fin_nblk, float fin_sc0,
                                                            float fin_sc1, float fin_alpha, float* __restrict__ fin_out,
                                                            const long long* __restrict__ n_valid) {
-  __shared__ float L[TP * LS], M[TP * LS];
+  constexpr bool HF = KIND == 2;
+  __shared__ __align__(16) float L1[TP * LS], M1[TP * MS], L2[HF ? TP * LS : 4], M2[HF ? TP * MS : 4];
   __shared__ double fin_w[4][2];
   const int tid = threadIdx.x, x0 = blockIdx.x * T, y0 = blockIdx.y * T;
-  const int tx = tid & 31, ty = tid >> 5;
+  const int vy = tid & 31, vq = tid >> 5;
   const size_t img = (size_t)blockIdx.z * H * W;
+  load_tiles<DECT, 1>({L1}, {r1 + (size_t)blockIdx.z * (H / 4) * (W / 4)}, H, W, y0, x0, tid);
+  if constexpr (HF) load_tiles<ZERO, 1>({L2}, {r2 + img}, H, W, y0, x0, tid);
+  __syncthreads();
+  hpass<true>(L1, M1, k1, 1.f, 0.f, x0, W, tid);
+  if constexpr (HF) hpass<true>(L2, M2, k2, 1.f, 0.f, x0, W, tid);
+  __syncthreads();
   float acc[4];
-  load_tile_dect(L, r1 + (size_t)blockIdx.z * (H / 4) * (W / 4), H, W, y0, x0, tid);
-  __syncthreads();
-  hpass_adj(L, M, k1, x0, W, tid);
-  __syncthreads();
-#pragma unroll
-  for (int r = 0; r < 4; ++r) acc[r] = vpass_adj_at(M, k1, ty + 8 * r, tx, y0, H);
-  __syncthreads();
-  if (KIND == 2) {
-    load_tile_zero(L, r2 + img, H, W, y0, x0, tid);
-    __syncthreads();
-    hpass_adj(L, M, k2, x0, W, tid);
-    __syncthreads();
-#pragma unroll
-    for (int r = 0; r < 4; ++r) {
-      const int y = ty + 8 * r;
-      acc[r] += L[(y + R) * LS + tx + R] - vpass_adj_at(M, k2, y, tx, y0, H);
-    }
+  vpass<true>(M1, k1, vy, vq, y0, H, acc);
+  if constexpr (HF) {
+    float g[4];
+    vpass<true>(M2, k2, vy, vq, y0, H, g);
+    const float4 c = ld4(L2 + (vy + R) * LS + 4 * vq + R);
+    acc[0] += c.x - g[0]; acc[1] += c.y - g[1]; acc[2] += c.z - g[2]; acc[3] += c.w - g[3];
   } else {
     const float F[4][9] = {{1, 2, 1, 0, 0, 0, -1, -2, -1}, {1, 0, -1, 2, 0, -2, 1, 0, -1},
                            {2, 1, 0, 1, 0, -1, 0, -1, -2}, {0, 1, 2, -1, 0, 1, -2, -1, 0}};
 #pragma unroll
-    for (int r = 0; r < 4; ++r) {
-      const int y = y0 + ty + 8 * r, x = x0 + tx;
+    for (int j = 0; j < 4; ++j) {
+      const int y = y0 + vy, x = x0 + 4 * vq + j;
       float s = 0.f;
 #pragma unroll
       for (int t = 0; t < 9; ++t) {
@@ -445,12 +462,10 @@
           s += F[0][t] * g.x + F[1][t] * g.y + F[2][t] * g.z + F[3][t] * g.w;
         }
       }
-      acc[r] += s;
-    }
-  }
-#pragma unroll
-  for (int r = 0; r < 4; ++r)
-    if (y0 + ty + 8 * r < H && x0 + tx < W) dsr[img + (size_t)(y0 + ty + 8 * r) * W + x0 + tx] = acc[r];
+      acc[j] += s;
+    }
+  }
+  if (y0 + vy < H) store_quad(dsr + img + (size_t)(y0 + vy) * W, x0 + 4 * vq, W, acc, aligned16(dsr + img));
   if (fin_out != nullptr && blockIdx.x == 0 && blockIdx.y == 0 && blockIdx.z == 0) {
     if constexpr (MASKED) masked_scales(n_valid, KIND == 1 ? 64.0 : 16.0, &fin_sc0, &fin_sc1);
     double s0 = 0.0, s1 = 0.0;
@@ -479,13 +494,13 @@
 
 int launch_blur_fwd(const float* x, const float* taps9, float* out, int B, int H, int W, hipStream_t s) {
   SIFSR_CHECK_ANY(H, W, 1);
-  hipLaunchKernelGGL(blur_fwd_kernel, SIFSR_TGRID(H, W, B), dim3(256), 0, s, x, out, make_taps(taps9), H, W);
+  hipLaunchKernelGGL(blur_kernel<REFLECT>, SIFSR_TGRID(H, W, B), dim3(256), 0, s, x, out, make_taps(taps9), H, W);
   SIFSR_LAUNCH_CHECK();
   return SIFSR_OK;
 }
 int launch_blur_bwd(const float* g, const float* taps9, float* out, int B, int H, int W, hipStream_t s) {
   SIFSR_CHECK_ANY(H, W, 1);
-  hipLaunchKernelGGL(blur_bwd_kernel, SIFSR_TGRID(H, W, B), dim3(256), 0, s, g, out, make_taps(taps9), H, W);
+  hipLaunchKernelGGL(blur_kernel<ZERO>, SIFSR_TGRID(H, W, B), dim3(256), 0, s, g, out, make_taps(taps9), H, W);
   SIFSR_LAUNCH_CHECK();
   return SIFSR_OK;
 }
@@ -497,7 +512,7 @@
 }
 int launch_blurdec_bwd(const float* glr, const float* taps9, float* out, int B, int H, int W, hipStream_t s) {
   SIFSR_CHECK_ANY(H, W, 4);
-  hipLaunchKernelGGL(blurdec_bwd_kernel, SIFSR_TGRID(H, W, B), dim3(256), 0, s, glr, out, make_taps(taps9), H, W);
+  hipLaunchKernelGGL(blur_kernel<DECT>, SIFSR_TGRID(H, W, B), dim3(256), 0, s, glr, out, make_taps(taps9), H, W);
   SIFSR_LAUNCH_CHECK();
   return SIFSR_OK;
 }
```
